# Nicolo2277/Vivim

Measured on AMD Instinct MI355X. Metric: frames/sec fwd+bwd, 256x256 clip=5 3-class, higher is better.
Workload: dtype bf16

## Files before the change

__graft_entry__.py:

```python
import os
import subprocess
import sys

ROOT = os.path.dirname(os.path.abspath(__file__))
if ROOT not in sys.path:
    sys.path.insert(0, ROOT)


def build() -> None:
    from vivim_amd import _lib
    _lib.build()
    subprocess.check_call(["make", "-C", os.path.join(ROOT, "oracle"), "-s"])
    L = _lib.lib()
    import re
    header = open(os.path.join(ROOT, "include", "vivim_hip.h")).read()
    assert L.vivim_abi_version() == int(re.search(r"#define VIVIM_ABI_VERSION (\d+)", header).group(1))
    import causal_conv1d
    import mamba_ssm
    import modeling.vivim


def smoke() -> None:
    import torch
    from mamba_ssm.ops.selective_scan_interface import mamba_inner_fn_no_out_proj
    from oracle import ref_torch
    assert torch.cuda.is_available(), "smoke() needs a GPU"
    dev = torch.device("cuda:0")
    g = torch.Generator().manual_seed(0)
    b, d_inner, n, r, L = 2, 128, 16, 4, 3 * 16 * 16
    p = dict(conv_w=torch.randn(d_inner, 1, 4, generator=g) * 0.3, conv_b=torch.randn(d_inner, generator=g) * 0.1,
             x_proj=torch.randn(r + 2 * n, d_inner, generator=g) * d_inner ** -0.5,
             dt_proj=(torch.rand(d_inner, r, generator=g) * 2 - 1) * r ** -0.5,
             A=-torch.arange(1, n + 1, dtype=torch.float32).repeat(d_inner, 1), D=torch.ones(d_inner),
             dt_bias=torch.full((d_inner,), -4.0))
    xz = torch.randn(b, 2 * d_inner, L, generator=g)
    dout = torch.randn(b, d_inner, L, generator=g)

    def run(device, fn):
        q = {k: v.to(device).requires_grad_(True) for k, v in p.items()}
        x = xz.to(device).requires_grad_(True)
        if fn is mamba_inner_fn_no_out_proj:
            y = fn(x, q["conv_w"], q["conv_b"], q["x_proj"], q["dt_proj"], q["A"], None, None, q["D"],
                   delta_bias=q["dt_bias"], delta_softplus=True)
        else:
            y = fn(x, q["conv_w"], q["conv_b"], q["x_proj"], q["dt_proj"], q["A"], q["D"], q["dt_bias"], True)
        y.backward(dout.to(device))
        return [y.detach().cpu(), x.grad.cpu()] + [q[k].grad.cpu() for k in sorted(q)]

    got = run(dev, mamba_inner_fn_no_out_proj)
    want = run("cpu", ref_torch.mamba_inner_no_out_proj_ref)
    for i, (a, w) in enumerate(zip(got, want)):
        err = float((a.double() - w.double()).norm() / w.double().norm())
        assert err < 1e-3, f"smoke: tensor {i} rel err {err:.3e}"
    torch.cuda.synchronize()
    print("smoke OK: fused inner op fwd+bwd matches the oracle (max rel err < 1e-3)")


if __name__ == "__main__":
    build()
    if len(sys.argv) > 1 and sys.argv[1] == "smoke":
        smoke()
```

vivim_amd/_lib.py:

```python
import collections
import ctypes
import os
import re
import subprocess

import torch

_HERE = os.path.dirname(os.path.abspath(__file__))
CSRC = os.path.join(_HERE, "csrc")
SO_PATH = os.environ.get("VIVIM_LIB") or os.path.join(CSRC, "libvivim_hip.so")
HEADER = os.path.join(os.path.dirname(_HERE), "include", "vivim_hip.h")
EXT_HEADER = os.path.join(os.path.dirname(_HERE), "include", "vivim_hip_ext.h")

i32, i64, vp = ctypes.c_int32, ctypes.c_int64, ctypes.c_void_p

STRUCT_NAMES = {
    "vivim_ssm_fwd_params": "SsmFwdParams", "vivim_ssm_bwd_params": "SsmBwdParams",
    "vivim_conv_fwd_params": "ConvFwdParams", "vivim_conv_bwd_params": "ConvBwdParams",
    "vivim_dwconv_params": "DwConvParams", "vivim_dwconv_wgrad_params": "DwConvWgradParams",
    "vivim_dir_params": "DirParams", "vivim_conv_update_params": "ConvUpdateParams",
    "vivim_state_update_params": "StateUpdateParams", "vivim_layernorm_params": "LayerNormParams",
    "vivim_wgrad_nt_params": "WgradNtParams", "vivim_add_layernorm_params": "AddLayerNormParams",
    "vivim_seg_loss_params": "SegLossParams", "vivim_seg_metrics_params": "SegMetricsParams",
    "vivim_upsample_params": "UpsampleParams",
    "vivim_decode_head_params": "DecodeHeadParams", "vivim_token_layernorm_params": "TokenLayerNormParams",
    "vivim_token_add_norm_params": "TokenAddNormParams", "vivim_opt_step_params": "OptStepParams",
    "vivim_opt_mw_params": "OptMwParams",
}
EXT_STRUCT_NAMES = {"vivim_structure_loss_params": "StructureLossParams"}
EXTENSIONS = {
    "vivim_hip_ext.h": (EXT_STRUCT_NAMES, {}),
    "vivim_hip_ext_head.h": ({"vivim_head_concat_params": "HeadConcatParams"}, {}),
}

Entry = collections.namedtuple("Entry", "struct extra stream restype")

_FIELD_TYPES = {"int32_t": i32, "int64_t": i64, "float": ctypes.c_float, "double": ctypes.c_double,
                "void *": vp, "const void *": vp, "const void *const *": ctypes.POINTER(vp),
                "const int64_t *": ctypes.POINTER(i64)}
_ARG_TYPES = {"void *": vp, "size_t": ctypes.c_size_t, "int": ctypes.c_int}
_RESTYPES = {"int": ctypes.c_int, "size_t": ctypes.c_size_t, "const char *": ctypes.c_char_p}
_DIRECTIVES = r"\s*#\s*(include|define|ifndef\s+VIVIM_HIP(_[A-Z0-9]+)*_H|endif)\b"


def _refuse(what, text):
    raise ValueError(f"vivim_hip.h: {what}: {' '.join(text.split())!r}")


def _ctype(text):
    return re.sub(r"\s*\*\s*", " *", " ".join(text.split()))


def _declarator(text, table, context):
    m = re.fullmatch(r"([\w\s*]*?)(\w+)\s*(?:\[\s*(\d+)\s*\])?", text.strip())
    if not m:
        _refuse("cannot parse the declarator", context)
    if _ctype(m[1]) not in table:
        _refuse(f"unknown type {_ctype(m[1])!r}", context)
    ctype = table[_ctype(m[1])]
    return m[2], (ctype * int(m[3]) if m[3] else ctype)


def _has_sizeof_row(cls):
    return cls._fields_[0][0] != "struct_bytes"


def parse_header(text, names=STRUCT_NAMES):
    text = re.sub(r"/\*.*?\*/", " ", text, flags=re.S)
    consts = {k: int(v) for k, v in re.findall(r"^[ \t]*#[ \t]*define[ \t]+(VIVIM_\w+)[ \t]+(-?\d+)[ \t]*$", text, flags=re.M)}
    by_c_name = {}

    def struct(m):
        body, c_name = m[1], m[2]
        if "{" in body or "#" in body:
            _refuse("nested braces or a preprocessor line in a struct", m[0])
        if c_name not in names:
            _refuse("a struct without a Python name in STRUCT_NAMES", c_name)
        types = {**_FIELD_TYPES, **by_c_name}
        fields = []
        for stmt in filter(None, (s.strip() for s in body.split(";"))):
            base = re.match(r"(?:const\s+)?\w+", stmt) or _refuse("cannot parse the field", stmt)
            first, *more = stmt.split(",")
            for decl in [first] + [f"{base[0]} {d}" for d in more]:
                fields.append(_declarator(decl, types, stmt))
        by_c_name[c_name] = type(names[c_name], (ctypes.Structure,), {"_fields_": fields, "__module__": __name__})
        return " "

    def enum(m):
        for item in filter(None, (s.strip() for s in m[1].split(","))):
            kv = re.fullmatch(r"(\w+)\s*=\s*(-?\d+)", item) or _refuse("cannot parse the enumerator", item)
            consts[kv[1]] = int(kv[2])
        return " "

    text = re.sub(r"typedef\s+struct\s*\{(.*?)\}\s*(\w+)\s*;", struct, text, flags=re.S)
    text = re.sub(r"(?:typedef\s+)?enum\s*\{([^{}]*)\}\s*\w*\s*;", enum, text)
    missing = [c for c in names if c not in by_c_name]
    if missing:
        _refuse("STRUCT_NAMES names structs the header does not have", ", ".join(missing))
    text = re.sub(r"^[ \t]*#[ \t]*ifdef[ \t]+__cplusplus\b.*?^[ \t]*#[ \t]*endif\b", " ", text, flags=re.S | re.M)
    for line in re.findall(r"^[ \t]*#.*$", text, flags=re.M):
        if not re.match(_DIRECTIVES, line):
            _refuse("a preprocessor line it does not know", line)
    text = re.sub(r"^[ \t]*#.*$", " ", text, flags=re.M)

    entries = {}
    for decl in filter(None, (s.strip() for s in text.split(";"))):
        m = re.fullmatch(r"([\w\s*]+?)(\w+)\s*\(([\w\s*,]*)\)", decl) or _refuse("cannot parse the declaration", decl)
        if _ctype(m[1]) not in _RESTYPES:
            _refuse(f"unknown return type {_ctype(m[1])!r}", decl)
        args = [] if m[3].strip() == "void" else [a.strip() for a in m[3].split(",")]
        stream = bool(args) and re.fullmatch(r"void\s*\*\s*stream", args[-1]) is not None
        args = args[:-1] if stream else args
        params, extra = None, []
        for k, arg in enumerate(args):
            p = re.fullmatch(r"const\s+(vivim_\w+)\s*\*\s*\w+", arg) if k == 0 else None
            if not p:
                extra.append(_declarator(arg, _ARG_TYPES, decl)[1])
            elif p[1] not in by_c_name:
                _refuse(f"unknown struct {p[1]}", decl)
            elif _has_sizeof_row(by_c_name[p[1]]):
                params = by_c_name[p[1]]
            else:
                extra.append(ctypes.POINTER(by_c_name[p[1]]))
        entries[m[2]] = Entry(params, tuple(extra), stream, _RESTYPES[_ctype(m[1])])
    return consts, {names[c]: by_c_name[c] for c in names}, entries


def _read_header(path=None):
    path = path or HEADER
    try:
        with open(path) as f:
            return f.read()
    except OSError as e:
        raise ImportError(f"{path} cannot be read ({e}): the binding is derived from it") from e


_consts, _classes, ENTRY_POINTS = parse_header(_read_header())
globals().update(_classes)
STRUCTS = tuple(c for c in _classes.values() if _has_sizeof_row(c))
EXPORTS = tuple(ENTRY_POINTS)
ABI_VERSION = _consts["VIVIM_ABI_VERSION"]
F32, F16, BF16 = _consts["VIVIM_F32"], _consts["VIVIM_F16"], _consts["VIVIM_BF16"]
OPT_CHUNK, OPT_MAX_TENSORS, OPT_STATE_WORDS = (_consts["VIVIM_OPT_" + n] for n in ("CHUNK", "MAX_TENSORS", "STATE_WORDS"))
ALL_ENTRY_POINTS = dict(ENTRY_POINTS)
for _file, (_names, _entries) in EXTENSIONS.items():
    _path = os.path.join(os.path.dirname(HEADER), _file)
    _, _ext_classes, _parsed = parse_header(_read_header(_path), _names)
    if any(_has_sizeof_row(c) for c in _ext_classes.values()) or set(_parsed) & set(ALL_ENTRY_POINTS) \
            or set(_ext_classes) & set(globals()):
        raise ImportError(f"{_path}: a struct that does not open with struct_bytes, or a name another header already declares")
    _entries.update(_parsed)
    ALL_ENTRY_POINTS.update(_parsed)
    globals().update(_ext_classes)
EXT_ENTRY_POINTS = EXTENSIONS[os.path.basename(EXT_HEADER)][1]

_lib = None


def build(force=False):
    if force:
        subprocess.check_call(["make", "-C", CSRC, "clean"])
    subprocess.check_call(["make", "-C", CSRC, "-j4"])
    return SO_PATH


def lib():
    global _lib
    if _lib is None:
        if not os.path.exists(SO_PATH):
            raise ImportError(
                f"{SO_PATH} is missing: run `python -c 'import __graft_entry__ as g; g.build()'` "
                "(or `make -C vivim_amd/csrc`). vivim_amd has no fallback path.")
        L = ctypes.CDLL(SO_PATH)
        for name, e in ALL_ENTRY_POINTS.items():
            fn = getattr(L, name)
            fn.argtypes = ([ctypes.POINTER(e.struct)] if e.struct else []) + list(e.extra) + ([vp] if e.stream else [])
            fn.restype = e.restype
        if L.vivim_abi_version() != ABI_VERSION:
            raise ImportError("libvivim_hip.so ABI version mismatch")
        for which, st in enumerate(STRUCTS):
            if L.vivim_sizeof(which) != ctypes.sizeof(st):
                raise ImportError(f"struct layout mismatch for {st.__name__}: "
                                  f"C {L.vivim_sizeof(which)} vs ctypes {ctypes.sizeof(st)}")
        _lib = L
    return _lib


_ISIZE = {F32: 4, F16: 2, BF16: 2}


def algorithmic_bytes(name, P):
    name = name.removesuffix("_det")
    f = P.f if isinstance(P, (SsmBwdParams, ConvBwdParams)) else P
    if name.startswith("vivim_opt"):
        if name.endswith("finalise"):
            return 8 * P.total_blocks + 4 * OPT_STATE_WORDS
        n = sum(P.numel[i] for i in range(P.count) if P.grads[i])
        if name.endswith("_mw"):
            return 2 * n + 8 * P.n_blocks if name.endswith("stats_mw") else 28 * n
        return 4 * n + 8 * P.n_blocks if name.endswith("stats") else 28 * n
    if name.startswith("vivim_add_layernorm"):
        n = P.batch * P.seqlen * P.channels
        if not P.weight:
            return n * ((2 if name.endswith("fwd") else 1) * _ISIZE[P.itype] + _ISIZE[P.btype])
        if name.endswith("fwd"):
            return n * (2 * _ISIZE[P.itype] + _ISIZE[P.btype] + _ISIZE[P.otype]) + 8 * P.batch * P.seqlen + 8 * P.channels
        res = (_ISIZE[P.itype] if P.dres else 0) + (_ISIZE[P.otype] if P.dy else 0) + (_ISIZE[P.btype] if P.dbranch else 0)
        return n * (2 * _ISIZE[P.itype] + res) + 8 * P.batch * P.seqlen + 12 * P.channels
    if name.startswith("vivim_token_add_norm"):
        n, b, r = P.rows * P.channels, _ISIZE[P.btype], _ISIZE[P.rtype]
        stats = 8 * P.rows if P.mean and P.weight else 0
        small = (4 * (P.rows // P.rows_per_sample) if P.scale else 0) + (4 * P.channels if P.weight else 0)
        if name.endswith("fwd"):
            small += 4 * P.channels if P.weight and P.bias else 0
            return n * (b + (r if P.res else 0) + (r if P.res_out else 0) + (b if P.weight else 0)) + stats + small
        norm = bool(P.weight and P.dy)
        small += (4 * P.channels if norm and P.dweight else 0) + (4 * P.channels if norm and P.dbias else 0)
        return (n * ((r + b if norm else 0) + (r if P.dres else 0) + (r if P.dres_in else 0) + (b if P.dbranch else 0))
                + (stats if norm else 0) + small)
    if name.startswith("vivim_token_layernorm"):
        n = P.rows * P.channels
        stats = 8 * P.rows if P.mean else 0
        if name.endswith("fwd"):
            return n * (_ISIZE[P.itype] + _ISIZE[P.otype]) + stats
        return n * (2 * _ISIZE[P.itype] + _ISIZE[P.otype]) + stats + 12 * P.channels
    if name.startswith("vivim_decode_head"):
        px = sum(P.map_h[s] * P.map_w[s] for s in range(P.n_maps))
        return (P.batch * (px * P.hidden + P.classes * P.out_h * P.out_w) * _ISIZE[P.itype]
                + 4 * (P.hidden + P.classes * P.hidden + P.classes))
    if name.startswith("vivim_head_concat"):
        px = P.out_h * P.out_w
        maps = sum(P.map_c[s] * (P.map_h[s] * P.map_w[s] + px) for s in range(P.n_maps)) * _ISIZE[P.itype]
        return P.batch * (maps + sum(P.map_c[s] * px for s in range(P.n_maps) if P.keep[s]))
    if name.startswith("vivim_upsample"):
        return P.batch * P.channels * (P.in_h * P.in_w + P.out_h * P.out_w) * _ISIZE[P.itype]
    if name.startswith("vivim_seg_metrics"):
        n = P.batch * P.pixels
        return n * (P.classes * _ISIZE[P.itype] + (8 if P.ttype == 0 else 1) + (1 if P.pred else 0)) + 12 * P.batch * P.classes
    if name.startswith("vivim_structure_loss"):
        n = P.batch * P.height * P.width
        return (n * ((2 if name.endswith("bwd") else 1) * P.classes * _ISIZE[P.itype] + (8 if P.ttype == 0 else 1))
                + 12 * P.batch * P.classes)
    if name.startswith("vivim_seg_loss"):
        n = P.batch * P.pixels
        return (n * ((2 if name.endswith("bwd") else 1) * P.classes * _ISIZE[P.itype] + (8 if P.ttype == 0 else 1))
                + 8 * P.batch * P.classes)
    if name.startswith("vivim_binary_metrics"):
        n = P.batch * P.height * P.width
        return (3 * n * (_ISIZE[P.ptype] + _ISIZE.get(P.gtype, 1)) + P.batch * (72 + (4096 if P.hist else 0))
                + (160 if P.state else 0))
    if name.startswith("vivim_selective_scan"):
        s = _ISIZE[f.itype]
        act = f.batch * f.dim * f.seqlen * s
        bc = (f.batch * f.n_groups * f.dstate * f.seqlen) if f.is_variable_B else f.dim * f.dstate
        has_z = bool(f.z)
        if name.endswith("fwd_lean"):
            return (4 if has_z else 3) * act + 2 * bc * (s if f.is_variable_B else 4) + 4 * (f.dim * f.dstate + 2 * f.dim)
        if name.endswith("fwd"):
            n_act = 3 + (2 if has_z else 0)
            return n_act * act + 2 * bc * (s if f.is_variable_B else 4) + 4 * (f.dim * f.dstate + 2 * f.dim)
        n_act = 5 + (3 if has_z else 0) + (1 if (has_z and f.out_z) else 0)
        return (n_act * act + 2 * bc * (s if f.is_variable_B else 4) + 2 * bc * 4
                + 4 * (2 * f.dim * f.dstate + 4 * f.dim))
    if name.endswith("_update"):
        return 0
    if name.startswith("vivim_dir"):
        return 4 * P.batch * P.channels * P.seqlen * _ISIZE[P.itype]
    if name.startswith("vivim_dwconv"):
        act = P.batch * P.depth * P.height * P.width * P.channels * _ISIZE[P.itype]
        return 2 * act + 4 * P.channels * (P.kd * 9 + 1)
    if name.startswith("vivim_layernorm"):
        n = P.batch * P.seqlen * P.channels
        if name.endswith("fwd"):
            return n * (_ISIZE[P.itype] + _ISIZE[P.otype]) + 8 * P.batch * P.seqlen + 8 * P.channels
        return n * (2 * _ISIZE[P.itype] + _ISIZE[P.otype]) + 8 * P.batch * P.seqlen + 12 * P.channels
    if name.startswith("vivim_wgrad"):
        return P.groups * ((P.m + P.n) * P.k * _ISIZE[P.itype] + 4 * P.m * P.n)
    s = _ISIZE[f.itype]
    act = f.batch * f.dim * f.seqlen * s
    if name.endswith("fwd"):
        return 2 * act + 4 * f.dim * (f.width + 1)
    return 3 * act + 8 * f.dim * (f.width + 1)


_profile = None
_event_pool = []
_PROFILED = ("vivim_selective_scan_fwd", "vivim_selective_scan_bwd", "vivim_causal_conv1d_fwd",
             "vivim_causal_conv1d_bwd")


def profile_begin(all_kernels=False):
    global _profile
    _profile = ([], bool(all_kernels))


def profile_end():
    global _profile
    rec = _profile[0] if _profile else []
    _profile = None
    out = []
    for name, nbytes, e0, e1 in rec:
        e1.synchronize()
        out.append((name, nbytes, e0.elapsed_time(e1) * 1e-3))
        _event_pool.extend((e0, e1))
    return out


def _event():
    if _event_pool:
        return _event_pool.pop()
    return torch.cuda.Event(enable_timing=True)


GUARD = os.environ.get("VIVIM_GUARD", "0") not in ("0", "")
_GUARD_BYTES = 1 << 16
_guards = []


def _guarded_storage(nbytes, device):
    buf = torch.full((nbytes + 2 * _GUARD_BYTES,), 0xA5, dtype=torch.uint8, device=device)
    _guards.append(buf)
    return buf[_GUARD_BYTES:_GUARD_BYTES + nbytes]


def empty(shape, dtype, device):
    if not GUARD:
        return torch.empty(shape, dtype=dtype, device=device)
    n = 1
    for d in shape:
        n *= d
    return _guarded_storage(n * torch.empty((), dtype=dtype).element_size(), device).view(dtype).view(shape)


def zeros(n, device):
    if not GUARD:
        return torch.zeros(n, dtype=torch.float32, device=device)
    return _guarded_storage(4 * n, device).view(torch.float32).zero_()


def empty_like(t):
    if not GUARD:
        return torch.empty_like(t)
    ref = torch.empty_like(t)
    flat = _guarded_storage(t.numel() * t.element_size(), t.device).view(t.dtype)
    return flat.as_strided(ref.shape, ref.stride())


def check_guards(what):
    torch.cuda.synchronize()
    for buf in _guards:
        lo, hi = buf[:_GUARD_BYTES], buf[-_GUARD_BYTES:]
        if not (bool((lo == 0xA5).all()) and bool((hi == 0xA5).all())):
            nlo, nhi = int((lo != 0xA5).sum()), int((hi != 0xA5).sum())
            _guards.clear()
            raise RuntimeError(f"VIVIM_GUARD: {what} wrote outside a {buf.numel() - 2 * _GUARD_BYTES}-byte buffer "
                               f"({nlo} bytes below, {nhi} bytes above)")
    _guards.clear()


def deterministic():
    return torch.are_deterministic_algorithms_enabled()


def call(name, params, stream, *extra):
    L = lib()
    fn = getattr(L, name)
    if _profile is not None and (_profile[1] or name in _PROFILED):
        e0, e1 = _event(), _event()
        e0.record()
        rc = fn(ctypes.byref(params), *extra, stream)
        e1.record()
        _profile[0].append((name, algorithmic_bytes(name, params), e0, e1))
    else:
        rc = fn(ctypes.byref(params), *extra, stream)
    if rc != 0:
        raise RuntimeError(L.vivim_last_error().decode())
    if GUARD:
        check_guards(name)


def launch(name, params, device, *extra):
    if device.index == torch.cuda.current_device():
        call(name, params, torch.cuda.current_stream().cuda_stream, *extra)
    else:
        with torch.cuda.device(device):
            call(name, params, torch.cuda.current_stream().cuda_stream, *extra)


ITYPE = {torch.float32: F32, torch.float16: F16, torch.bfloat16: BF16}


def ptr(t):
    return None if t is None else t.data_ptr()


def check(cond, msg):
    if not cond:
        raise RuntimeError(msg)


def workspace(query, params, device):
    n = getattr(lib(), query)(params)
    return n, (empty((n,), torch.uint8, device) if n else None)
```

vivim_amd/csrc/capi.hip:

```cpp
#include <hip/hip_runtime.h>
#include <float.h>
#include <stdarg.h>
#include <stddef.h>
#include <stdio.h>
#include <string.h>
#include <type_traits>
#include "ops.cuh"

using vivim::Launch;
using vivim::conv_channel_last;
using vivim::elem_bytes;
using vivim::vec_elems;

static thread_local char g_err[512] = "";

static int fail(int code, const char* fmt, ...) {
    va_list ap;
    va_start(ap, fmt);
    vsnprintf(g_err, sizeof(g_err), fmt, ap);
    va_end(ap);
    return code;
}

#define VCHECK(cond)                                                                   \
    do {                                                                               \
        if (!(cond)) return fail(VIVIM_ERR_INVALID, "%s: check failed: %s", __func__, #cond); \
    } while (0)

static int after_launch(const char* what) {
    const hipError_t e = hipGetLastError();
    if (e != hipSuccess) return fail(VIVIM_ERR_LAUNCH, "%s: launch failed: %s", what, hipGetErrorString(e));
    return VIVIM_OK;
}

static bool dtype_ok(int t) { return t == VIVIM_F32 || t == VIVIM_F16 || t == VIVIM_BF16; }
static bool aligned(const void* q, uintptr_t bytes) { return reinterpret_cast<uintptr_t>(q) % bytes == 0; }
static bool aligned16(const void* q) { return aligned(q, 16); }
static hipStream_t as_stream(void* stream) { return static_cast<hipStream_t>(stream); }

static int bad_workspace(const char* fn, const char* query, long long bytes, const void* at, int align, size_t need) {
    return fail(VIVIM_ERR_INVALID, "%s: workspace of %lld bytes at %p: need a %d-byte aligned one of %s() = %zu", fn, bytes, at, align,
                query, need);
}
static int check_workspace(const char* fn, const char* query, const void* ws, int64_t bytes, int align, size_t need) {
    if (ws == nullptr || !aligned(ws, align) || bytes < 0 || (size_t)bytes < need) return bad_workspace(fn, query, bytes, ws, align, need);
    return VIVIM_OK;
}
static int check_struct_bytes(const char* fn, const char* name, int32_t struct_bytes, size_t size) {
    if (struct_bytes != (int32_t)size)
        return fail(VIVIM_ERR_INVALID, "%s: struct_bytes = %d, this library's %s has %zu", fn, struct_bytes, name, size);
    return VIVIM_OK;
}

enum SsmCheck { kSsmFwd, kSsmBwd, kSsmFwdLean };
static int check_ssm_fwd(const vivim_ssm_fwd_params* p, SsmCheck mode) {
    const bool is_bwd = mode == kSsmBwd;
    VCHECK(p != nullptr);
    VCHECK(dtype_ok(p->itype));
    VCHECK(p->batch > 0 && p->dim > 0 && p->seqlen > 0 && p->dstate > 0 && p->n_groups > 0);
    VCHECK(p->dstate <= 256);
    VCHECK(p->dim % p->n_groups == 0);
    VCHECK(p->u && p->delta && p->A && p->B && p->C);
    if (mode == kSsmFwdLean) {
        if (p->x != nullptr)
            return fail(VIVIM_ERR_INVALID, "selective_scan_fwd_lean: x must be NULL (this entry point writes no checkpoints; "
                        "vivim_selective_scan_fwd is the call that fills x)");
        if (p->z) {
            VCHECK(p->out_z != nullptr);
            if (p->out != nullptr)
                return fail(VIVIM_ERR_INVALID, "selective_scan_fwd_lean: with z only out_z is written, out must be NULL");
        } else {
            VCHECK(p->out != nullptr);
        }
    } else {
        VCHECK(p->x != nullptr || (is_bwd && p->seqlen <= vivim::scan_ckpt_len(*p)));
        if (!is_bwd) VCHECK(p->out != nullptr);
        if (p->z) {
            if (!is_bwd) VCHECK(p->out_z != nullptr);
            else VCHECK(p->out != nullptr);
        }
    }
    if (p->is_variable_B != p->is_variable_C)
        return fail(VIVIM_ERR_UNSUPPORTED,
                    "selective_scan: mixed constant/variable B and C is not built (Vivim uses variable B and C)");
    if (!p->is_variable_B) VCHECK(p->n_groups == 1);
    return VIVIM_OK;
}

template <class P> static int check_seg_inputs(const P* p, const char* name) {
    VCHECK(p != nullptr);
    VCHECK(dtype_ok(p->itype) && (p->ttype == 0 || p->ttype == 1));
    VCHECK(p->batch > 0 && p->pixels > 0);
    if (p->classes < 2 || p->classes > 8)
        return fail(VIVIM_ERR_UNSUPPORTED, "%s: %d classes: the kernels are built for 2 to 8 classes", name, p->classes);
    if constexpr (std::is_same<P, vivim_seg_loss_params>::value)
        if (p->gamma != 2.0f)
            return fail(VIVIM_ERR_UNSUPPORTED, "seg_loss: gamma = %g: the kernels are built for gamma = 2 only", (double)p->gamma);
    VCHECK((int64_t)p->batch * 64 <= INT32_MAX);
    VCHECK(p->logits && aligned(p->logits, p->itype == VIVIM_F32 ? 4 : 2));
    VCHECK(p->target && aligned(p->target, p->ttype == 0 ? 8 : 1));
    return VIVIM_OK;
}

namespace vivim {
static int g_tune[2] = {-1, -1};
static int tuning_get(int which, const char* env) {
    int v = __atomic_load_n(&g_tune[which], __ATOMIC_RELAXED);
    if (v < 0) {
        const char* e = getenv(env);
        v = e ? atoi(e) : 0;
        if (v < 0) v = 0;
        __atomic_store_n(&g_tune[which], v, __ATOMIC_RELAXED);
    }
    return v;
}
int tuning_fwd_variant() { return tuning_get(0, "VIVIM_FWD_VARIANT"); }
int tuning_bwd_variant() { return tuning_get(1, "VIVIM_BWD_VARIANT"); }
}

extern "C" {

int vivim_set_tuning(int which, int value) {
    if (which < 0 || which > 1 || value < 0) return -1;
    const int prev = which == 0 ? vivim::tuning_fwd_variant() : vivim::tuning_bwd_variant();
    __atomic_store_n(&vivim::g_tune[which], value, __ATOMIC_RELAXED);
    return prev;
}
int vivim_abi_version(void) { return VIVIM_ABI_VERSION; }
const char* vivim_last_error(void) { return g_err; }
int vivim_scan_chunk_len(int itype) { return vivim::scan_chunk_len(itype); }
int vivim_scan_ckpt_len(const vivim_ssm_fwd_params* f) { return f ? vivim::scan_ckpt_len(*f) : 0; }
size_t vivim_scan_bwd_workspace_bytes(const vivim_ssm_fwd_params* f) {
    return f ? vivim::scan_bwd_workspace_bytes(*f) : 0;
}
size_t vivim_scan_fwd_workspace_bytes(const vivim_ssm_fwd_params* f) {
    return f ? vivim::scan_fwd_workspace_bytes(*f) : 0;
}
size_t vivim_sizeof(int which) {
    static const size_t sizes[] = {
        sizeof(vivim_ssm_fwd_params), sizeof(vivim_ssm_bwd_params), sizeof(vivim_conv_fwd_params), sizeof(vivim_conv_bwd_params),
        sizeof(vivim_dwconv_params), sizeof(vivim_dwconv_wgrad_params), sizeof(vivim_dir_params), sizeof(vivim_conv_update_params),
        sizeof(vivim_state_update_params), sizeof(vivim_layernorm_params), sizeof(vivim_wgrad_nt_params),
        sizeof(vivim_add_layernorm_params), sizeof(vivim_seg_loss_params), sizeof(vivim_seg_metrics_params),
        sizeof(vivim_upsample_params)};
    return which >= 0 && which < (int)(sizeof(sizes) / sizeof(sizes[0])) ? sizes[which] : 0;
}

int vivim_selective_scan_fwd(const vivim_ssm_fwd_params* p, void* stream) {
    if (int rc = check_ssm_fwd(p, kSsmFwd)) return rc;
    if (!vivim::ssm_fwd_dispatch(*p, as_stream(stream)))
        return fail(VIVIM_ERR_UNSUPPORTED, "selective_scan_fwd not implemented for input type %d", p->itype);
    return after_launch("selective_scan_fwd");
}

int vivim_selective_scan_fwd_lean(const vivim_ssm_fwd_params* p, void* last_state, void* stream) {
    if (int rc = check_ssm_fwd(p, kSsmFwdLean)) return rc;
    if (!vivim::ssm_fwd_lean_dispatch(*p, last_state, as_stream(stream)))
        return fail(VIVIM_ERR_UNSUPPORTED, "selective_scan_fwd_lean not implemented for input type %d", p->itype);
    return after_launch("selective_scan_fwd_lean");
}

static int check_ssm_bwd(const vivim_ssm_bwd_params* p) {
    VCHECK(p != nullptr);
    if (int rc = check_ssm_fwd(&p->f, kSsmBwd)) return rc;
    VCHECK(p->dout && p->du && p->ddelta && p->dA && p->dB && p->dC);
    VCHECK((p->f.D == nullptr) == (p->dD == nullptr));
    VCHECK((p->f.delta_bias == nullptr) == (p->ddelta_bias == nullptr));
    VCHECK((p->f.z == nullptr) == (p->dz == nullptr));
    return VIVIM_OK;
}

int vivim_selective_scan_bwd(const vivim_ssm_bwd_params* p, void* stream) {
    if (int rc = check_ssm_bwd(p)) return rc;
    if (!vivim::ssm_bwd_dispatch(*p, as_stream(stream)))
        return fail(VIVIM_ERR_UNSUPPORTED, "selective_scan_bwd not implemented for input type %d", p->f.itype);
    return after_launch("selective_scan_bwd");
}

size_t vivim_scan_bwd_det_workspace_bytes(const vivim_ssm_fwd_params* f) {
    return f && f->batch > 0 && f->dim > 0 && f->seqlen > 0 && f->dstate > 0 && f->n_groups > 0
               ? vivim::scan_bwd_det_workspace_bytes(*f) : 0;
}

size_t vivim_scan_bwd_det_call_workspace_bytes(const vivim_ssm_bwd_params* p) {
    return check_ssm_bwd(p) == VIVIM_OK ? vivim::scan_bwd_det_call_workspace_bytes(*p) : 0;
}

int vivim_selective_scan_bwd_det(const vivim_ssm_bwd_params* p, void* det_ws, size_t det_ws_bytes, void* stream) {
    if (int rc = check_ssm_bwd(p)) return rc;
    switch (vivim::ssm_bwd_det_dispatch(*p, det_ws, det_ws_bytes, as_stream(stream))) {
        case Launch::ok: break;
        case Launch::bad_workspace:
            return bad_workspace("selective_scan_bwd_det", "vivim_scan_bwd_det_call_workspace_bytes", det_ws_bytes, det_ws, 16,
                                 vivim::scan_bwd_det_call_workspace_bytes(*p));
        case Launch::unsupported: return fail(VIVIM_ERR_UNSUPPORTED, "selective_scan_bwd_det not implemented for input type %d", p->f.itype);
    }
    return after_launch("selective_scan_bwd_det");
}

static int check_conv(const vivim_conv_fwd_params* p) {
    VCHECK(p != nullptr);
    VCHECK(dtype_ok(p->itype) && dtype_ok(p->wtype));
    VCHECK(p->batch > 0 && p->dim > 0 && p->seqlen > 0);
    VCHECK(p->batch <= 65535 && p->dim <= 65535);
    if (!(p->width >= 2 && p->width <= 4))
        return fail(VIVIM_ERR_INVALID, "causal_conv1d only supports width between 2 and 4");
    VCHECK(p->x && p->weight);
    if (p->x_l_stride != 1 && p->x_c_stride != 1)
        return fail(VIVIM_ERR_INVALID, "causal_conv1d: x must have unit stride along seqlen or along channels");
    return VIVIM_OK;
}

int vivim_causal_conv1d_fwd(const vivim_conv_fwd_params* p, void* stream) {
    if (int rc = check_conv(p)) return rc;
    VCHECK(p->out != nullptr);
    const bool cl = conv_channel_last(*p);
    if (cl) { VCHECK(p->out_c_stride == 1); } else { VCHECK(p->out_l_stride == 1); }
    if (!vivim::conv_fwd_dispatch(*p, as_stream(stream)))
        return fail(VIVIM_ERR_UNSUPPORTED, "causal_conv1d_fwd not implemented for input type %d / weight type %d",
                    p->itype, p->wtype);
    return after_launch("causal_conv1d_fwd");
}

static int check_conv_bwd(const vivim_conv_bwd_params* p) {
    VCHECK(p != nullptr);
    if (int rc = check_conv(&p->f)) return rc;
    VCHECK(p->dout && p->dx && p->dweight);
    const bool cl = conv_channel_last(p->f);
    if (cl) { VCHECK(p->dout_c_stride == 1 && p->dx_c_stride == 1); }
    else    { VCHECK(p->dout_l_stride == 1 && p->dx_l_stride == 1); }
    VCHECK((p->f.bias == nullptr) == (p->dbias == nullptr));
    return VIVIM_OK;
}

size_t vivim_causal_conv1d_bwd_det_workspace_bytes(const vivim_conv_fwd_params* f) {
    return check_conv(f) == VIVIM_OK ? vivim::conv_bwd_det_workspace_bytes(*f) : 0;
}

int vivim_causal_conv1d_bwd_det(const vivim_conv_bwd_params* p, void* det_ws, size_t det_ws_bytes, void* stream) {
    if (int rc = check_conv_bwd(p)) return rc;
    switch (vivim::conv_bwd_det_dispatch(*p, det_ws, det_ws_bytes, as_stream(stream))) {
        case Launch::ok: break;
        case Launch::bad_workspace:
            return bad_workspace("causal_conv1d_bwd_det", "vivim_causal_conv1d_bwd_det_workspace_bytes", det_ws_bytes, det_ws, 16,
                                 vivim::conv_bwd_det_workspace_bytes(p->f));
        case Launch::unsupported:
            return fail(VIVIM_ERR_UNSUPPORTED, "causal_conv1d_bwd_det not implemented for input type %d / weight type %d",
                        p->f.itype, p->f.wtype);
    }
    return after_launch("causal_conv1d_bwd_det");
}

int vivim_causal_conv1d_bwd(const vivim_conv_bwd_params* p, void* stream) {
    if (int rc = check_conv_bwd(p)) return rc;
    if (!vivim::conv_bwd_dispatch(*p, as_stream(stream)))
        return fail(VIVIM_ERR_UNSUPPORTED, "causal_conv1d_bwd not implemented for input type %d / weight type %d",
                    p->f.itype, p->f.wtype);
    return after_launch("causal_conv1d_bwd");
}

static int check_dw_dims(int batch, int depth, int height, int width, int channels, int kd, int itype) {
    VCHECK(dtype_ok(itype));
    VCHECK(batch > 0 && depth > 0 && height > 0 && width > 0 && channels > 0);
    VCHECK(kd == 1 || kd == 3);
    VCHECK(batch <= 65535);
    return VIVIM_OK;
}

int vivim_dwconv_fwd(const vivim_dwconv_params* p, void* stream) {
    VCHECK(p != nullptr);
    if (int rc = check_dw_dims(p->batch, p->depth, p->height, p->width, p->channels, p->kd, p->itype)) return rc;
    VCHECK(p->x && p->wt && p->y);
    const int64_t cv = vec_elems(p->itype);
    VCHECK(p->channels % cv == 0 && p->x_token_stride % cv == 0 && p->x_batch_stride % cv == 0 &&
           p->y_token_stride % cv == 0 && p->y_batch_stride % cv == 0);
    VCHECK(aligned16(p->x) && aligned16(p->y));
    VCHECK(p->act >= 0 && p->act <= 2 && (p->act == 0 || p->flip == 0));
    if (p->act == 2)
        VCHECK(p->aux && aligned16(p->aux) && p->aux_token_stride % cv == 0 &&
               p->aux_batch_stride % cv == 0);
    if (!vivim::dwconv_fwd_dispatch(*p, as_stream(stream)))
        return fail(VIVIM_ERR_UNSUPPORTED, "dwconv_fwd not implemented for input type %d", p->itype);
    return after_launch("dwconv_fwd");
}

static int check_dw_wgrad(const vivim_dwconv_wgrad_params* p) {
    VCHECK(p != nullptr);
    if (int rc = check_dw_dims(p->batch, p->depth, p->height, p->width, p->channels, p->kd, p->itype)) return rc;
    VCHECK(p->x && p->dy && p->dwt);
    VCHECK(p->channels % 2 == 0 && p->x_token_stride % 2 == 0 && p->x_batch_stride % 2 == 0 &&
           p->dy_token_stride % 2 == 0 && p->dy_batch_stride % 2 == 0);
    VCHECK(aligned(p->x, 8) && aligned(p->dy, 8));
    return VIVIM_OK;
}

size_t vivim_dwconv_wgrad_det_workspace_bytes(const vivim_dwconv_wgrad_params* p) {
    if (!p || p->batch <= 0 || p->depth <= 0 || p->height <= 0 || p->width <= 0 || p->channels <= 0 || (p->kd != 1 && p->kd != 3))
        return 0;
    return vivim::dwconv_wgrad_det_workspace_bytes(*p);
}

int vivim_dwconv_wgrad_det(const vivim_dwconv_wgrad_params* p, void* det_ws, size_t det_ws_bytes, void* stream) {
    if (int rc = check_dw_wgrad(p)) return rc;
    switch (vivim::dwconv_wgrad_det_dispatch(*p, det_ws, det_ws_bytes, as_stream(stream))) {
        case Launch::ok: break;
        case Launch::bad_workspace:
            return bad_workspace("dwconv_wgrad_det", "vivim_dwconv_wgrad_det_workspace_bytes", det_ws_bytes, det_ws, 16,
                                 vivim::dwconv_wgrad_det_workspace_bytes(*p));
        case Launch::unsupported: return fail(VIVIM_ERR_UNSUPPORTED, "dwconv_wgrad_det not implemented for input type %d", p->itype);
    }
    return after_launch("dwconv_wgrad_det");
}

int vivim_dwconv_wgrad(const vivim_dwconv_wgrad_params* p, void* stream) {
    if (int rc = check_dw_wgrad(p)) return rc;
    if (!vivim::dwconv_wgrad_dispatch(*p, as_stream(stream)))
        return fail(VIVIM_ERR_UNSUPPORTED, "dwconv_wgrad not implemented for input type %d", p->itype);
    return after_launch("dwconv_wgrad");
}

static int check_dir(const vivim_dir_params* p) {
    VCHECK(p != nullptr);
    VCHECK(p->itype == VIVIM_F32 || p->itype == VIVIM_F16 || p->itype == VIVIM_BF16);
    VCHECK(p->batch > 0 && p->channels > 0 && p->seqlen > 0 && p->nframes > 0 && p->csplit > 0);
    VCHECK(p->batch <= 65535 && p->channels <= 65535);
    VCHECK(p->seqlen % p->nframes == 0 && p->channels % p->csplit == 0);
    VCHECK(p->src && p->dst);
    const int64_t e = vec_elems(p->itype);
    VCHECK(p->seqlen % e == 0);
    VCHECK(aligned16(p->src) && aligned16(p->dst));
    VCHECK(p->flat_batch_stride % e == 0 && p->flat_c_stride % e == 0 && p->stk_batch_stride % e == 0 &&
           p->stk_half_stride % e == 0 && p->stk_dir_stride % e == 0 && p->stk_c_stride % e == 0);
    return VIVIM_OK;
}

int vivim_dir_scatter(const vivim_dir_params* p, void* stream) {
    if (int rc = check_dir(p)) return rc;
    if (!vivim::dir_dispatch<false>(*p, as_stream(stream))) return fail(VIVIM_ERR_UNSUPPORTED, "dir_scatter: bad itype");
    return after_launch("dir_scatter");
}

int vivim_dir_gather(const vivim_dir_params* p, void* stream) {
    if (int rc = check_dir(p)) return rc;
    if (!vivim::dir_dispatch<true>(*p, as_stream(stream))) return fail(VIVIM_ERR_UNSUPPORTED, "dir_gather: bad itype");
    return after_launch("dir_gather");
}

int vivim_causal_conv1d_update(const vivim_conv_update_params* p, void* stream) {
    VCHECK(p != nullptr);
    VCHECK(dtype_ok(p->itype) && dtype_ok(p->wtype));
    VCHECK(p->batch > 0 && p->dim > 0 && p->batch <= 65535);
    if (p->width < 2 || p->width > 4)
        return fail(VIVIM_ERR_UNSUPPORTED, "causal_conv1d only supports width between 2 and 4");
    VCHECK(p->x && p->conv_state && p->weight && p->out);
    vivim::conv_update_launch(*p, as_stream(stream));
    return after_launch("causal_conv1d_update");
}

int vivim_selective_state_update(const vivim_state_update_params* p, void* stream) {
    VCHECK(p != nullptr);
    VCHECK(dtype_ok(p->itype) && (p->stype == VIVIM_F32 || p->stype == p->itype));
    VCHECK(p->batch > 0 && p->dim > 0 && p->dstate > 0 && p->batch <= 65535);
    VCHECK(p->state && p->x && p->dt && p->A && p->B && p->C && p->out);
    vivim::state_update_launch(*p, as_stream(stream));
    return after_launch("selective_state_update");
}

static int check_layernorm(const vivim_layernorm_params* p) {
    VCHECK(p != nullptr);
    VCHECK(dtype_ok(p->itype) && (p->otype == VIVIM_F32 || p->otype == p->itype));
    VCHECK(p->batch > 0 && p->seqlen > 0 && p->channels > 0 && p->batch <= 65535);
    if (p->channels > 512)
        return fail(VIVIM_ERR_UNSUPPORTED, "layernorm_cm: more than 512 channels do not fit the backward's two LDS tiles");
    const int64_t e = vec_elems(p->itype);
    VCHECK(p->seqlen % e == 0 && p->x_batch_stride % e == 0 && p->x_c_stride % e == 0);
    VCHECK(p->x && aligned16(p->x) && p->mean && p->rstd);
    return VIVIM_OK;
}

int vivim_layernorm_cm_fwd(const vivim_layernorm_params* p, void* stream) {
    if (int rc = check_layernorm(p)) return rc;
    VCHECK(p->y != nullptr);
    if (!vivim::layernorm_dispatch(*p, false, as_stream(stream)))
        return fail(VIVIM_ERR_UNSUPPORTED, "layernorm_cm_fwd not implemented for input type %d / output type %d", p->itype, p->otype);
    return after_launch("layernorm_cm_fwd");
}

size_t vivim_layernorm_bwd_workspace_bytes(const vivim_layernorm_params* p) {
    return p && p->batch > 0 && p->seqlen > 0 && p->channels > 0 ? vivim::layernorm_bwd_workspace_bytes(*p) : 0;
}

int vivim_layernorm_cm_bwd(const vivim_layernorm_params* p, void* stream) {
    if (int rc = check_layernorm(p)) return rc;
    VCHECK(p->dy && p->dx && aligned16(p->dx));
    const int64_t e = vec_elems(p->itype);
    VCHECK(p->dx_batch_stride % e == 0 && p->dx_c_stride % e == 0);
    if ((p->dweight || p->dbias) && !p->workspace)
        return fail(VIVIM_ERR_INVALID, "layernorm_cm_bwd: dweight / dbias need the workspace (vivim_layernorm_bwd_workspace_bytes)");
    if (!vivim::layernorm_dispatch(*p, true, as_stream(stream)))
        return fail(VIVIM_ERR_UNSUPPORTED, "layernorm_cm_bwd not implemented for input type %d / output type %d", p->itype, p->otype);
    return after_launch("layernorm_cm_bwd");
}

int vivim_wgrad_nt(const vivim_wgrad_nt_params* p, void* stream) {
    VCHECK(p != nullptr);
    VCHECK(p->groups > 0 && p->groups <= 65535 && p->m > 0 && p->n > 0 && p->k > 0);
    VCHECK(p->a && p->b && p->out);
    if (p->itype != VIVIM_F16 && p->itype != VIVIM_BF16)
        return fail(VIVIM_ERR_UNSUPPORTED, "wgrad_nt takes f16 or bf16 operands (type %d given): f32 products stay on the library GEMM", p->itype);
    VCHECK(p->k % 8 == 0 && p->a_row_stride % 8 == 0 && p->b_row_stride % 8 == 0 && p->a_group_stride % 8 == 0 &&
           p->b_group_stride % 8 == 0);
    VCHECK(aligned16(p->a) && aligned16(p->b));
    VCHECK((int64_t)((p->m + 63) / 64) * ((p->n + 15) / 16) <= 65535);
    if (!vivim::wgrad_nt_dispatch(*p, as_stream(stream)))
        return fail(VIVIM_ERR_UNSUPPORTED, "wgrad_nt not implemented for type %d", p->itype);
    return after_launch("wgrad_nt");
}

static int check_add_layernorm(const vivim_add_layernorm_params* p, int64_t* e) {
    VCHECK(p != nullptr);
    VCHECK(dtype_ok(p->itype) && dtype_ok(p->btype) && (p->weight == nullptr || dtype_ok(p->otype)));
    VCHECK(p->batch > 0 && p->seqlen > 0 && p->channels > 0 && p->batch <= 65535);
    if (p->channels > 512)
        return fail(VIVIM_ERR_UNSUPPORTED, "add_layernorm_cm: more than 512 channels do not fit the backward's two LDS tiles");
    if (p->btype != p->itype && p->itype != VIVIM_F32)
        return fail(VIVIM_ERR_UNSUPPORTED, "add_layernorm_cm: branch type %d with x type %d is not built (the branch has x's type, or x is f32)",
                    p->btype, p->itype);
    if (p->weight && p->otype != VIVIM_F32 && p->otype != p->itype)
        return fail(VIVIM_ERR_UNSUPPORTED, "add_layernorm_cm: output type %d with x type %d is not built (f32 or x's type)", p->otype, p->itype);
    *e = vec_elems(p->itype);
    VCHECK(p->seqlen % *e == 0);
    return VIVIM_OK;
}

int vivim_add_layernorm_cm_fwd(const vivim_add_layernorm_params* p, void* stream) {
    int64_t e = 0;
    if (int rc = check_add_layernorm(p, &e)) return rc;
    VCHECK(p->x && p->branch && p->x_new && aligned16(p->x) && aligned16(p->x_new));
    VCHECK(p->x_batch_stride % e == 0 && p->x_c_stride % e == 0 && p->x_new_batch_stride % e == 0 && p->x_new_c_stride % e == 0);
    if (p->weight) VCHECK(p->y && p->mean && p->rstd);
    if (!vivim::add_layernorm_dispatch(*p, false, as_stream(stream)))
        return fail(VIVIM_ERR_UNSUPPORTED, "add_layernorm_cm_fwd not implemented for x type %d / branch type %d / output type %d", p->itype,
                    p->btype, p->otype);
    return after_launch("add_layernorm_cm_fwd");
}

size_t vivim_add_layernorm_bwd_workspace_bytes(const vivim_add_layernorm_params* p) {
    return p && p->batch > 0 && p->seqlen > 0 && p->channels > 0 ? vivim::add_layernorm_bwd_workspace_bytes(*p) : 0;
}

int vivim_add_layernorm_cm_bwd(const vivim_add_layernorm_params* p, void* stream) {
    int64_t e = 0;
    if (int rc = check_add_layernorm(p, &e)) return rc;
    if (p->dres) VCHECK(aligned16(p->dres) && p->dres_batch_stride % e == 0 && p->dres_c_stride % e == 0);
    if (p->weight) {
        VCHECK(p->x_new && aligned16(p->x_new) && p->mean && p->rstd && (p->dy || p->dres));
        VCHECK(p->x_new_batch_stride % e == 0 && p->x_new_c_stride % e == 0);
        VCHECK(p->dx && aligned16(p->dx) && p->dx_batch_stride % e == 0 && p->dx_c_stride % e == 0);
        if ((p->dweight || p->dbias) && !p->workspace)
            return fail(VIVIM_ERR_INVALID,
                        "add_layernorm_cm_bwd: dweight / dbias need the workspace (vivim_add_layernorm_bwd_workspace_bytes)");
    } else {
        VCHECK(p->dres && p->dbranch);
    }
    if (!vivim::add_layernorm_dispatch(*p, true, as_stream(stream)))
        return fail(VIVIM_ERR_UNSUPPORTED, "add_layernorm_cm_bwd not implemented for x type %d / branch type %d / output type %d", p->itype,
                    p->btype, p->otype);
    return after_launch("add_layernorm_cm_bwd");
}

static int check_seg_loss(const vivim_seg_loss_params* p) {
    if (int rc = check_seg_inputs(p, "seg_loss")) return rc;
    VCHECK(p->alpha && aligned(p->alpha, 4));
    return VIVIM_OK;
}

size_t vivim_seg_loss_workspace_bytes(const vivim_seg_loss_params* p) {
    return p && p->batch > 0 && p->pixels > 0 && p->classes > 0 && dtype_ok(p->itype) ? vivim::seg_loss_workspace_bytes(*p) : 0;
}

int vivim_seg_loss_fwd(const vivim_seg_loss_params* p, void* stream) {
    if (int rc = check_seg_loss(p)) return rc;
    VCHECK(p->loss && aligned(p->loss, 4));
    VCHECK(aligned(p->coef, 4));
    const size_t need = vivim::seg_loss_workspace_bytes(*p);
    if (int rc = check_workspace("seg_loss_fwd", "vivim_seg_loss_workspace_bytes", p->workspace, p->workspace_bytes, 4, need)) return rc;
    if (!vivim::seg_loss_dispatch(*p, false, as_stream(stream)))
        return fail(VIVIM_ERR_UNSUPPORTED, "seg_loss_fwd not implemented for input type %d / %d classes", p->itype, p->classes);
    return after_launch("seg_loss_fwd");
}

int vivim_seg_loss_bwd(const vivim_seg_loss_params* p, void* stream) {
    if (int rc = check_seg_loss(p)) return rc;
    const uintptr_t ib = elem_bytes(p->itype);
    VCHECK(p->coef && aligned(p->coef, 4));
    VCHECK(p->grad_out && aligned(p->grad_out, 4));
    VCHECK(p->dlogits && aligned(p->dlogits, ib));
    if (!vivim::seg_loss_dispatch(*p, true, as_stream(stream)))
        return fail(VIVIM_ERR_UNSUPPORTED, "seg_loss_bwd not implemented for input type %d / %d classes", p->itype, p->classes);
    return after_launch("seg_loss_bwd");
}

size_t vivim_seg_metrics_workspace_bytes(const vivim_seg_metrics_params* p) {
    return p && p->batch > 0 && p->pixels > 0 && p->classes > 0 && dtype_ok(p->itype) ? vivim::seg_metrics_workspace_bytes(*p) : 0;
}

int vivim_seg_metrics(const vivim_seg_metrics_params* p, void* stream) {
    if (int rc = check_seg_inputs(p, "seg_metrics")) return rc;
    VCHECK(p->counts && aligned(p->counts, 4));
    VCHECK(aligned(p->state, 8));
    const size_t need = vivim::seg_metrics_workspace_bytes(*p);
    if (int rc = check_workspace("seg_metrics", "vivim_seg_metrics_workspace_bytes", p->workspace, p->workspace_bytes, 4, need)) return rc;
    if (!vivim::seg_metrics_dispatch(*p, as_stream(stream)))
        return fail(VIVIM_ERR_UNSUPPORTED, "seg_metrics not implemented for input type %d / %d classes", p->itype, p->classes);
    return after_launch("seg_metrics");
}

static int check_upsample(const vivim_upsample_params* p, bool bwd) {
    VCHECK(p != nullptr);
    VCHECK(dtype_ok(p->itype) && (p->layout == 0 || p->layout == 1));
    VCHECK(p->batch > 0 && p->channels > 0 && p->in_h > 0 && p->in_w > 0 && p->out_h > 0 && p->out_w > 0);
    if (p->out_h < p->in_h || p->out_w < p->in_w)
        return fail(VIVIM_ERR_UNSUPPORTED, "upsample_bilinear2d: (%d, %d) -> (%d, %d): upsampling only", p->in_h, p->in_w, p->out_h,
                    p->out_w);
    const uintptr_t ib = elem_bytes(p->itype);
    const void* src = bwd ? p->dy : p->x;
    const void* dst = bwd ? p->dx : p->y;
    VCHECK(src != nullptr && aligned(src, ib));
    VCHECK(dst != nullptr && aligned(dst, ib));
    VCHECK((int64_t)p->channels * p->in_h * p->in_w <= INT32_MAX && (int64_t)p->channels * p->out_h * p->out_w <= INT32_MAX);
    VCHECK((2 * (int64_t)p->in_h + 3) * p->out_h <= INT32_MAX && (2 * (int64_t)p->in_w + 3) * p->out_w <= INT32_MAX);
    VCHECK((int64_t)p->batch * p->channels <= INT32_MAX && (int64_t)p->batch * p->out_h <= INT32_MAX);
    VCHECK(vivim::upsample_blocks(*p, bwd) <= INT32_MAX);
    return VIVIM_OK;
}

int vivim_upsample_bilinear2d_fwd(const vivim_upsample_params* p, void* stream) {
    if (int rc = check_upsample(p, false)) return rc;
    if (!vivim::upsample_dispatch(*p, false, as_stream(stream)))
        return fail(VIVIM_ERR_UNSUPPORTED, "upsample_bilinear2d_fwd not implemented for type %d", p->itype);
    return after_launch("upsample_bilinear2d_fwd");
}

int vivim_upsample_bilinear2d_bwd(const vivim_upsample_params* p, void* stream) {
    if (int rc = check_upsample(p, true)) return rc;
    if (!vivim::upsample_dispatch(*p, true, as_stream(stream)))
        return fail(VIVIM_ERR_UNSUPPORTED, "upsample_bilinear2d_bwd not implemented for type %d", p->itype);
    return after_launch("upsample_bilinear2d_bwd");
}

static int check_decode_head(const vivim_decode_head_params* p) {
    VCHECK(p != nullptr);
    if (int rc = check_struct_bytes("decode_head_fwd", "vivim_decode_head_params", p->struct_bytes, sizeof(*p))) return rc;
    VCHECK(dtype_ok(p->itype));
    VCHECK(p->batch > 0 && p->hidden > 0 && p->classes > 0 && p->out_h > 0 && p->out_w > 0);
    VCHECK(p->n_maps >= 1 && p->n_maps <= 4);
    VCHECK(p->classes <= 8);
    if (p->hidden > vivim::decode_head_max_hidden())
        return fail(VIVIM_ERR_INVALID, "decode_head_fwd: hidden = %d: bias and w_out are kept in LDS, which holds up to %d channels",
                    p->hidden, vivim::decode_head_max_hidden());
    const uintptr_t ib = elem_bytes(p->itype);
    VCHECK((int64_t)p->classes * p->out_h * p->out_w <= INT32_MAX);
    for (int s = 0; s < p->n_maps; ++s) {
        VCHECK(p->map_h[s] > 0 && p->map_w[s] > 0);
        if (p->map_h[s] > p->out_h || p->map_w[s] > p->out_w)
            return fail(VIVIM_ERR_UNSUPPORTED, "decode_head_fwd: map %d is (%d, %d), the output (%d, %d): upsampling only", s, p->map_h[s],
                        p->map_w[s], p->out_h, p->out_w);
        VCHECK((int64_t)p->hidden * p->map_h[s] * p->map_w[s] <= INT32_MAX);
    }
    for (int s = 0; s < p->n_maps; ++s) VCHECK(p->maps[s] != nullptr && aligned(p->maps[s], ib));
    VCHECK(p->bias != nullptr && aligned(p->bias, 4));
    VCHECK(p->w_out != nullptr && aligned(p->w_out, 4));
    VCHECK(aligned(p->b_out, 4));
    VCHECK(p->logits != nullptr && aligned(p->logits, ib));
    for (int s = 0; s < p->n_maps; ++s) VCHECK(p->map_batch_stride[s] >= (int64_t)p->hidden * p->map_h[s] * p->map_w[s]);
    VCHECK(p->logits_batch_stride >= (int64_t)p->classes * p->out_h * p->out_w);
    VCHECK(vivim::decode_head_blocks(*p) <= INT32_MAX);
    return VIVIM_OK;
}

int vivim_decode_head_fwd(const vivim_decode_head_params* p, void* stream) {
    if (int rc = check_decode_head(p)) return rc;
    if (!vivim::decode_head_dispatch(*p, as_stream(stream)))
        return fail(VIVIM_ERR_UNSUPPORTED, "decode_head_fwd not implemented for type %d", p->itype);
    return after_launch("decode_head_fwd");
}

static int check_token_layernorm(const vivim_token_layernorm_params* p, const char* fn) {
    VCHECK(p != nullptr);
    if (int rc = check_struct_bytes(fn, "vivim_token_layernorm_params", p->struct_bytes, sizeof(*p))) return rc;
    VCHECK(dtype_ok(p->itype) && dtype_ok(p->otype));
    VCHECK(p->rows > 0);
    if (p->channels < 1)
        return fail(VIVIM_ERR_INVALID, "%s: channels = %d: a row has at least one channel", fn, p->channels);
    if (p->channels > 1024)
        return fail(VIVIM_ERR_UNSUPPORTED, "%s: channels = %d: a row of more than 1024 channels does not fit the lanes' registers", fn,
                    p->channels);
    if (!vivim::token_layernorm_pair_ok(p->itype, p->otype))
        return fail(VIVIM_ERR_UNSUPPORTED, "%s: input type %d with output type %d is not built (the same type, an f32 output, or an f32 input)",
                    fn, p->itype, p->otype);
    VCHECK(p->x != nullptr && aligned(p->x, p->itype == VIVIM_F32 ? 4 : 2));
    VCHECK(p->weight != nullptr && aligned(p->weight, 4));
    if (p->x_row_stride < p->channels)
        return fail(VIVIM_ERR_INVALID, "%s: x_row_stride = %lld is less than the %d channels of a row", fn, (long long)p->x_row_stride,
                    p->channels);
    return VIVIM_OK;
}

int vivim_token_layernorm_fwd(const vivim_token_layernorm_params* p, void* stream) {
    if (int rc = check_token_layernorm(p, "token_layernorm_fwd")) return rc;
    VCHECK(p->y != nullptr && aligned(p->y, p->otype == VIVIM_F32 ? 4 : 2));
    VCHECK(aligned(p->bias, 4));
    VCHECK((p->mean == nullptr) == (p->rstd == nullptr) && aligned(p->mean, 4) && aligned(p->rstd, 4));
    if (p->y_row_stride < p->channels)
        return fail(VIVIM_ERR_INVALID, "token_layernorm_fwd: y_row_stride = %lld is less than the %d channels of a row",
                    (long long)p->y_row_stride, p->channels);
    if (!vivim::token_layernorm_dispatch(*p, false, as_stream(stream)))
        return fail(VIVIM_ERR_UNSUPPORTED, "token_layernorm_fwd not implemented for input type %d / output type %d", p->itype, p->otype);
    return after_launch("token_layernorm_fwd");
}

size_t vivim_token_layernorm_bwd_workspace_bytes(const vivim_token_layernorm_params* p) {
    return p && p->rows > 0 && p->channels > 0 && p->channels <= 1024 ? vivim::token_layernorm_bwd_workspace_bytes(*p) : 0;
}

int vivim_token_layernorm_bwd(const vivim_token_layernorm_params* p, void* stream) {
    if (int rc = check_token_layernorm(p, "token_layernorm_bwd")) return rc;
    VCHECK(p->dy != nullptr && aligned(p->dy, p->otype == VIVIM_F32 ? 4 : 2));
    VCHECK(p->dx != nullptr && aligned(p->dx, p->itype == VIVIM_F32 ? 4 : 2));
    VCHECK(p->mean != nullptr && p->rstd != nullptr && aligned(p->mean, 4) && aligned(p->rstd, 4));
    VCHECK(aligned(p->dweight, 4) && aligned(p->dbias, 4) && aligned(p->workspace, 4));
    if (p->dy_row_stride < p->channels || p->dx_row_stride < p->channels)
        return fail(VIVIM_ERR_INVALID, "token_layernorm_bwd: dy_row_stride = %lld / dx_row_stride = %lld is less than the %d channels of a row",
                    (long long)p->dy_row_stride, (long long)p->dx_row_stride, p->channels);
    if ((p->dweight || p->dbias) && !p->workspace)
        return fail(VIVIM_ERR_INVALID, "token_layernorm_bwd: dweight / dbias need the workspace (vivim_token_layernorm_bwd_workspace_bytes)");
    if (!vivim::token_layernorm_dispatch(*p, true, as_stream(stream)))
        return fail(VIVIM_ERR_UNSUPPORTED, "token_layernorm_bwd not implemented for input type %d / output type %d", p->itype, p->otype);
    return after_launch("token_layernorm_bwd");
}

static int check_token_add_norm(const vivim_token_add_norm_params* p, const char* fn) {
    VCHECK(p != nullptr);
    if (int rc = check_struct_bytes(fn, "vivim_token_add_norm_params", p->struct_bytes, sizeof(*p))) return rc;
    if (!dtype_ok(p->btype) || !dtype_ok(p->rtype) || !dtype_ok(p->otype))
        return fail(VIVIM_ERR_INVALID, "%s: btype = %d, rtype = %d, otype = %d: a type tag is 0 (f32), 1 (f16) or 2 (bf16)", fn, p->btype,
                    p->rtype, p->otype);
    if (p->rows <= 0) return fail(VIVIM_ERR_INVALID, "%s: rows = %d: at least one row", fn, p->rows);
    if (p->channels < 1)
        return fail(VIVIM_ERR_INVALID, "%s: channels = %d: a row has at least one channel", fn, p->channels);
    if (p->channels > 1024)
        return fail(VIVIM_ERR_UNSUPPORTED, "%s: channels = %d: a row of more than 1024 channels does not fit the lanes' registers", fn,
                    p->channels);
    if (!vivim::token_add_norm_pair_ok(p->btype, p->rtype) || p->otype != p->btype)
        return fail(VIVIM_ERR_UNSUPPORTED, "%s: branch type %d with residual type %d and output type %d is not built (one type, or an "
                    "f16 / bf16 branch and output on an f32 residual)", fn, p->btype, p->rtype, p->otype);
    if (p->rms != 0 && p->rms != 1) return fail(VIVIM_ERR_INVALID, "%s: rms = %d: 0 (LayerNorm) or 1 (RMSNorm)", fn, p->rms);
    if (p->scale != nullptr && (p->rows_per_sample <= 0 || p->rows % p->rows_per_sample != 0))
        return fail(VIVIM_ERR_INVALID, "%s: rows_per_sample = %d with scale: it must be positive and divide rows = %d", fn,
                    p->rows_per_sample, p->rows);
    return VIVIM_OK;
}

static int check_tan_tensor(const char* fn, const char* name, const void* q, bool required, int type, int64_t stride, int channels) {
    if (q == nullptr)
        return required ? fail(VIVIM_ERR_INVALID, "%s: %s is NULL", fn, name) : VIVIM_OK;
    if (!aligned(q, elem_bytes(type)))
        return fail(VIVIM_ERR_INVALID, "%s: %s = %p is not aligned to its element type", fn, name, q);
    if (stride < channels)
        return fail(VIVIM_ERR_INVALID, "%s: %s_row_stride = %lld is less than the %d channels of a row", fn, name, (long long)stride, channels);
    return VIVIM_OK;
}
static int check_tan_f32(const char* fn, const char* name, const void* q, bool required) {
    if (q == nullptr)
        return required ? fail(VIVIM_ERR_INVALID, "%s: %s is NULL", fn, name) : VIVIM_OK;
    return aligned(q, 4) ? VIVIM_OK : fail(VIVIM_ERR_INVALID, "%s: %s = %p is not aligned to its element type", fn, name, q);
}

int vivim_token_add_norm_fwd(const vivim_token_add_norm_params* p, void* stream) {
    const char* fn = "token_add_norm_fwd";
    if (int rc = check_token_add_norm(p, fn)) return rc;
    const bool norm = p->weight != nullptr;
    const int C = p->channels;
    if (int rc = check_tan_tensor(fn, "branch", p->branch, true, p->btype, p->branch_row_stride, C)) return rc;
    if (int rc = check_tan_tensor(fn, "res", p->res, false, p->rtype, p->res_row_stride, C)) return rc;
    if (int rc = check_tan_tensor(fn, "res_out", p->res_out, !norm || p->res != nullptr, p->rtype, p->res_out_row_stride, C)) return rc;
    if (int rc = check_tan_f32(fn, "scale", p->scale, false)) return rc;
    if (norm) {
        if (int rc = check_tan_tensor(fn, "y", p->y, true, p->otype, p->y_row_stride, C)) return rc;
        if (int rc = check_tan_f32(fn, "weight", p->weight, true)) return rc;
        if (int rc = check_tan_f32(fn, "bias", p->bias, false)) return rc;
        if ((p->mean == nullptr) != (p->rstd == nullptr))
            return fail(VIVIM_ERR_INVALID, "%s: mean = %p with rstd = %p: both or neither", fn, p->mean, p->rstd);
        if (int rc = check_tan_f32(fn, "mean", p->mean, false)) return rc;
        if (int rc = check_tan_f32(fn, "rstd", p->rstd, false)) return rc;
    }
    if (!vivim::token_add_norm_dispatch(*p, false, as_stream(stream)))
        return fail(VIVIM_ERR_UNSUPPORTED, "%s not implemented for branch type %d / residual type %d", fn, p->btype, p->rtype);
    return after_launch(fn);
}

size_t vivim_token_add_norm_bwd_workspace_bytes(const vivim_token_add_norm_params* p) {
    return p && p->rows > 0 && p->channels > 0 && p->channels <= 1024 ? vivim::token_add_norm_bwd_workspace_bytes(*p) : 0;
}

int vivim_token_add_norm_bwd(const vivim_token_add_norm_params* p, void* stream) {
    const char* fn = "token_add_norm_bwd";
    if (int rc = check_token_add_norm(p, fn)) return rc;
    const bool norm = p->weight != nullptr;
    const int C = p->channels;
    if (p->dy == nullptr && p->dres == nullptr) return fail(VIVIM_ERR_INVALID, "%s: dy and dres are both NULL: nothing to propagate", fn);
    if (!norm && p->dy != nullptr) return fail(VIVIM_ERR_INVALID, "%s: dy = %p without weight: the add alone has no y", fn, p->dy);
    if (norm) {
        if (int rc = check_tan_tensor(fn, "res_out", p->res_out, true, p->rtype, p->res_out_row_stride, C)) return rc;
        if (int rc = check_tan_f32(fn, "mean", p->mean, true)) return rc;
        if (int rc = check_tan_f32(fn, "rstd", p->rstd, true)) return rc;
        if (int rc = check_tan_f32(fn, "weight", p->weight, true)) return rc;
        if (int rc = check_tan_tensor(fn, "dy", p->dy, false, p->otype, p->dy_row_stride, C)) return rc;
        if (int rc = check_tan_f32(fn, "dweight", p->dweight, false)) return rc;
        if (int rc = check_tan_f32(fn, "dbias", p->dbias, false)) return rc;
        if (int rc = check_tan_f32(fn, "workspace", p->workspace, false)) return rc;
        if ((p->dweight || p->dbias) && !p->workspace)
            return fail(VIVIM_ERR_INVALID, "%s: dweight / dbias need the workspace (vivim_token_add_norm_bwd_workspace_bytes)", fn);
    }
    if (int rc = check_tan_tensor(fn, "dres", p->dres, false, p->rtype, p->dres_row_stride, C)) return rc;
    if (int rc = check_tan_tensor(fn, "dres_in", p->dres_in, false, p->rtype, p->dres_in_row_stride, C)) return rc;
    if (int rc = check_tan_tensor(fn, "dbranch", p->dbranch, false, p->btype, p->dbranch_row_stride, C)) return rc;
    if (int rc = check_tan_f32(fn, "scale", p->scale, false)) return rc;
    if (!vivim::token_add_norm_dispatch(*p, true, as_stream(stream)))
        return fail(VIVIM_ERR_UNSUPPORTED, "%s not implemented for branch type %d / residual type %d", fn, p->btype, p->rtype);
    return after_launch(fn);
}

static int check_opt_common(const vivim_opt_step_params* p, const char* fn) {
    VCHECK(p != nullptr);
    if (int rc = check_struct_bytes(fn, "vivim_opt_step_params", p->struct_bytes, sizeof(*p))) return rc;
    VCHECK(p->state != nullptr && aligned(p->state, 4));
    if (p->total_blocks < 0) return fail(VIVIM_ERR_INVALID, "%s: total_blocks = %d", fn, p->total_blocks);
    return VIVIM_OK;
}

static int check_opt_tensors(const vivim_opt_step_params* p, const char* fn, size_t grad_align = 4) {
    if (p->count <= 0 || p->count > VIVIM_OPT_MAX_TENSORS)
        return fail(VIVIM_ERR_INVALID, "%s: count = %d, a call takes 1 to %d tensors", fn, p->count, VIVIM_OPT_MAX_TENSORS);
    VCHECK(p->grads != nullptr && p->numel != nullptr && p->block_map != nullptr);
    VCHECK(aligned(p->block_map, 4) && p->first_tensor >= 0);
    for (int i = 0; i < p->count; ++i) {
        if (p->numel[i] <= 0) return fail(VIVIM_ERR_INVALID, "%s: numel[%d] = %lld", fn, i, (long long)p->numel[i]);
        VCHECK(aligned(p->grads[i], grad_align));
    }
    if (p->first_block < 0 || p->n_blocks <= 0 || (int64_t)p->first_block + p->n_blocks > p->total_blocks)
        return fail(VIVIM_ERR_INVALID, "%s: map rows %d .. %d + %d of %d", fn, p->first_block, p->first_block, p->n_blocks, p->total_blocks);
    return VIVIM_OK;
}

static int check_opt_workspace(const vivim_opt_step_params* p, const char* fn) {
    const size_t need = 8 * (size_t)p->total_blocks;
    if (need && (p->workspace == nullptr || !aligned(p->workspace, 8) || p->workspace_bytes < (int64_t)need))
        return bad_workspace(fn, "vivim_opt_step_workspace_bytes", (long long)p->workspace_bytes, p->workspace, 8, need);
    return VIVIM_OK;
}

static int check_opt_hyper(const vivim_opt_step_params* p, const char* fn, bool update) {
    if (!(p->beta1 >= 0.0 && p->beta1 < 1.0 && p->beta2 >= 0.0 && p->beta2 < 1.0))
        return fail(VIVIM_ERR_INVALID, "%s: betas = (%g, %g), each must be in [0, 1)", fn, p->beta1, p->beta2);
    if (update && !(p->lr >= 0.0 && p->eps >= 0.0 && p->weight_decay >= 0.0))
        return fail(VIVIM_ERR_INVALID, "%s: lr = %g, eps = %g, weight_decay = %g: none may be negative", fn, p->lr, p->eps, p->weight_decay);
    return VIVIM_OK;
}

size_t vivim_opt_step_workspace_bytes(const vivim_opt_step_params* p) {
    return p && p->struct_bytes == (int32_t)sizeof(vivim_opt_step_params) && p->total_blocks > 0 ? 8 * (size_t)p->total_blocks : 0;
}

int vivim_opt_grad_stats(const vivim_opt_step_params* p, void* stream) {
    const char* fn = "opt_grad_stats";
    if (int rc = check_opt_common(p, fn)) return rc;
    if (int rc = check_opt_tensors(p, fn)) return rc;
    if (int rc = check_opt_workspace(p, fn)) return rc;
    vivim::opt_grad_stats_launch(*p, as_stream(stream));
    return after_launch(fn);
}

int vivim_opt_finalise(const vivim_opt_step_params* p, void* stream) {
    const char* fn = "opt_finalise";
    if (int rc = check_opt_common(p, fn)) return rc;
    if (int rc = check_opt_hyper(p, fn, false)) return rc;
    if (p->has_max_norm && !(p->max_norm >= 0.0)) return fail(VIVIM_ERR_INVALID, "%s: max_norm = %g", fn, p->max_norm);
    if (int rc = check_opt_workspace(p, fn)) return rc;
    vivim::opt_finalise_launch(*p, as_stream(stream));
    return after_launch(fn);
}

int vivim_opt_adamw(const vivim_opt_step_params* p, void* stream) {
    const char* fn = "opt_adamw";
    if (int rc = check_opt_common(p, fn)) return rc;
    VCHECK(p->params != nullptr && p->exp_avg != nullptr && p->exp_avg_sq != nullptr);
    VCHECK(aligned(p->params, 8) && aligned(p->exp_avg, 8) && aligned(p->exp_avg_sq, 8));
    if (int rc = check_opt_tensors(p, fn)) return rc;
    if (int rc = check_opt_hyper(p, fn, true)) return rc;
    vivim::opt_adamw_launch(*p, as_stream(stream));
    return after_launch(fn);
}

static int check_opt_mw(const vivim_opt_mw_params* p, const char* fn, vivim_opt_step_params& q) {
    VCHECK(p != nullptr);
    if (int rc = check_struct_bytes(fn, "vivim_opt_mw_params", p->struct_bytes, sizeof(*p))) return rc;
    static_assert(offsetof(vivim_opt_mw_params, masters) == sizeof(vivim_opt_step_params), "the common fields come first");
    memcpy(&q, p, sizeof(q));
    q.struct_bytes = (int32_t)sizeof(q);
    if (int rc = check_opt_common(&q, fn)) return rc;
    if (p->dtype != VIVIM_F16 && p->dtype != VIVIM_BF16)
        return fail(VIVIM_ERR_INVALID, "%s: dtype = %d, master weights are for 1 (fp16) and 2 (bf16)", fn, p->dtype);
    return VIVIM_OK;
}

int vivim_opt_grad_stats_mw(const vivim_opt_mw_params* p, void* stream) {
    const char* fn = "opt_grad_stats_mw";
    vivim_opt_step_params q;
    if (int rc = check_opt_mw(p, fn, q)) return rc;
    if (int rc = check_opt_tensors(&q, fn, 2)) return rc;
    if (int rc = check_opt_workspace(&q, fn)) return rc;
    vivim::opt_grad_stats_mw_launch(q, p->dtype, as_stream(stream));
    return after_launch(fn);
}

int vivim_opt_adamw_mw(const vivim_opt_mw_params* p, void* stream) {
    const char* fn = "opt_adamw_mw";
    vivim_opt_step_params q;
    if (int rc = check_opt_mw(p, fn, q)) return rc;
    VCHECK(q.params != nullptr && q.exp_avg != nullptr && q.exp_avg_sq != nullptr && p->masters != nullptr);
    VCHECK(aligned(q.params, 8) && aligned(q.exp_avg, 8) && aligned(q.exp_avg_sq, 8) && aligned(p->masters, 8));
    if (int rc = check_opt_tensors(&q, fn, 2)) return rc;
    if (int rc = check_opt_hyper(&q, fn, true)) return rc;
    vivim::opt_adamw_mw_launch(q, p->masters, p->dtype, as_stream(stream));
    return after_launch(fn);
}


static bool structure_loss_sizes_ok(const vivim_structure_loss_params* p) {
    return p->batch > 0 && p->classes > 0 && p->height > 0 && p->width > 0;
}

static int check_structure_loss(const vivim_structure_loss_params* p, const char* fn) {
    if (p == nullptr) return fail(VIVIM_ERR_INVALID, "%s: params is NULL", fn);
    if (int rc = check_struct_bytes(fn, "vivim_structure_loss_params", p->struct_bytes, sizeof(*p))) return rc;
    if (!dtype_ok(p->itype) || (p->ttype != 0 && p->ttype != 1))
        return fail(VIVIM_ERR_INVALID, "%s: itype = %d, ttype = %d: logits are fp32 / fp16 / bf16 (0 / 1 / 2), targets int64 / uint8 (0 / 1)",
                    fn, p->itype, p->ttype);
    if (!structure_loss_sizes_ok(p))
        return fail(VIVIM_ERR_INVALID, "%s: batch = %d, classes = %d, height = %d, width = %d: every size must be positive", fn, p->batch,
                    p->classes, p->height, p->width);
    if (p->classes > 8)
        return fail(VIVIM_ERR_UNSUPPORTED, "%s: %d classes: the kernels are built for 1 to 8 classes", fn, p->classes);
    if (p->first_class < 0 || p->first_class > 255)
        return fail(VIVIM_ERR_INVALID, "%s: first_class = %d: labels are compared as values in [0, 256)", fn, p->first_class);
    if ((int64_t)p->height * p->width > INT32_MAX - 4096 || (int64_t)p->batch * vivim::structure_loss_tiles(*p) > INT32_MAX)
        return fail(VIVIM_ERR_INVALID, "%s: batch = %d, height = %d, width = %d: the index range overflows int32", fn, p->batch, p->height,
                    p->width);
    const uintptr_t ib = elem_bytes(p->itype);
    if (p->logits == nullptr || !aligned(p->logits, ib))
        return fail(VIVIM_ERR_INVALID, "%s: logits at %p: need a %d-byte aligned pointer", fn, p->logits, (int)ib);
    if (p->target == nullptr || !aligned(p->target, p->ttype == 0 ? 8 : 1))
        return fail(VIVIM_ERR_INVALID, "%s: target at %p: need a %d-byte aligned pointer", fn, p->target, p->ttype == 0 ? 8 : 1);
    return VIVIM_OK;
}

size_t vivim_structure_loss_workspace_bytes(const vivim_structure_loss_params* p) {
    if (p == nullptr || p->struct_bytes != (int32_t)sizeof(vivim_structure_loss_params) || !structure_loss_sizes_ok(p) || p->classes > 8 ||
        !dtype_ok(p->itype))
        return 0;
    return vivim::structure_loss_workspace_bytes(*p);
}

int vivim_structure_loss_fwd(const vivim_structure_loss_params* p, void* stream) {
    const char* fn = "structure_loss_fwd";
    if (int rc = check_structure_loss(p, fn)) return rc;
    if (p->loss == nullptr || !aligned(p->loss, 4)) return fail(VIVIM_ERR_INVALID, "%s: loss at %p: need a 4-byte aligned pointer", fn, p->loss);
    if (!aligned(p->coef, 4))
        return fail(VIVIM_ERR_INVALID, "%s: coef at %p: need a 4-byte aligned pointer (or NULL)", fn, p->coef);
    const size_t need = vivim::structure_loss_workspace_bytes(*p);
    if (int rc = check_workspace(fn, "vivim_structure_loss_workspace_bytes", p->workspace, p->workspace_bytes, 8, need)) return rc;
    if (!vivim::structure_loss_dispatch(*p, false, as_stream(stream)))
        return fail(VIVIM_ERR_UNSUPPORTED, "%s not implemented for input type %d", fn, p->itype);
    return after_launch(fn);
}

int vivim_structure_loss_bwd(const vivim_structure_loss_params* p, void* stream) {
    const char* fn = "structure_loss_bwd";
    if (int rc = check_structure_loss(p, fn)) return rc;
    const uintptr_t ib = elem_bytes(p->itype);
    if (p->coef == nullptr || !aligned(p->coef, 4)) return fail(VIVIM_ERR_INVALID, "%s: coef at %p: need a 4-byte aligned pointer", fn, p->coef);
    if (p->grad_out == nullptr || !aligned(p->grad_out, 4))
        return fail(VIVIM_ERR_INVALID, "%s: grad_out at %p: need a 4-byte aligned pointer", fn, p->grad_out);
    if (p->dlogits == nullptr || !aligned(p->dlogits, ib))
        return fail(VIVIM_ERR_INVALID, "%s: dlogits at %p: need a %d-byte aligned pointer", fn, p->dlogits, (int)ib);
    if (!vivim::structure_loss_dispatch(*p, true, as_stream(stream)))
        return fail(VIVIM_ERR_UNSUPPORTED, "%s not implemented for input type %d", fn, p->itype);
    return after_launch(fn);
}


static int check_head_concat(const vivim_head_concat_params* p, const char* fn, bool bwd) {
    if (p == nullptr) return fail(VIVIM_ERR_INVALID, "%s: params is NULL", fn);
    if (int rc = check_struct_bytes(fn, "vivim_head_concat_params", p->struct_bytes, sizeof(*p))) return rc;
    if (p->n_maps < 1 || p->n_maps > 4) return fail(VIVIM_ERR_INVALID, "%s: n_maps = %d: one to four maps", fn, p->n_maps);
    if (!dtype_ok(p->itype)) return fail(VIVIM_ERR_INVALID, "%s: itype = %d: the maps are fp32 / fp16 / bf16 (0 / 1 / 2)", fn, p->itype);
    if (p->batch <= 0 || p->out_h <= 0 || p->out_w <= 0)
        return fail(VIVIM_ERR_INVALID, "%s: batch = %d, out_h = %d, out_w = %d: every size must be positive", fn, p->batch, p->out_h, p->out_w);
    for (int s = 0; s < p->n_maps; ++s)
        if (p->map_c[s] <= 0 || p->map_h[s] <= 0 || p->map_w[s] <= 0)
            return fail(VIVIM_ERR_INVALID, "%s: map %d: map_c = %d, map_h = %d, map_w = %d: every size must be positive", fn, s, p->map_c[s],
                        p->map_h[s], p->map_w[s]);
    for (int s = 0; s < p->n_maps; ++s)
        if (p->map_h[s] > p->out_h || p->map_w[s] > p->out_w)
            return fail(VIVIM_ERR_UNSUPPORTED, "%s: map %d is (%d, %d), the output (%d, %d): upsampling only", fn, s, p->map_h[s], p->map_w[s],
                        p->out_h, p->out_w);
    for (int s = 0; s < p->n_maps; ++s) {
        if (p->chan_off[s] < 0 || (int64_t)p->chan_off[s] + p->map_c[s] > p->out_pixel_stride)
            return fail(VIVIM_ERR_INVALID, "%s: map %d: channels [%d, %lld) lie outside a pixel of out_pixel_stride = %lld", fn, s, p->chan_off[s],
                        (long long)p->chan_off[s] + p->map_c[s], (long long)p->out_pixel_stride);
        for (int t = 0; t < s; ++t)
            if (p->chan_off[s] < p->chan_off[t] + p->map_c[t] && p->chan_off[t] < p->chan_off[s] + p->map_c[s])
                return fail(VIVIM_ERR_INVALID, "%s: the channel blocks of maps %d and %d overlap: [%d, %d) and [%d, %d)", fn, t, s, p->chan_off[t],
                            p->chan_off[t] + p->map_c[t], p->chan_off[s], p->chan_off[s] + p->map_c[s]);
    }
    const uintptr_t ib = elem_bytes(p->itype);
    const void* big = bwd ? p->dout : p->out;
    if (big == nullptr || !aligned(big, ib))
        return fail(VIVIM_ERR_INVALID, "%s: %s at %p: need a %d-byte aligned pointer", fn, bwd ? "dout" : "out", big, (int)ib);
    for (int s = 0; s < p->n_maps; ++s) {
        const void* q = bwd ? p->dmaps[s] : p->maps[s];
        if (q == nullptr || !aligned(q, ib))
            return fail(VIVIM_ERR_INVALID, "%s: %s[%d] at %p: need a %d-byte aligned pointer", fn, bwd ? "dmaps" : "maps", s, q, (int)ib);
    }
    for (int s = 0; s < p->n_maps; ++s)
        if (!(p->scale[s] >= 1.0f) || p->scale[s] > FLT_MAX)
            return fail(VIVIM_ERR_INVALID, "%s: scale[%d] = %g: 1 / (1 - p) is finite and at least 1", fn, s, (double)p->scale[s]);
    const int64_t out_image = (int64_t)p->out_h * p->out_w * p->out_pixel_stride;
    if (p->out_batch_stride < out_image)
        return fail(VIVIM_ERR_INVALID, "%s: out_batch_stride = %lld: an image of out has %lld elements", fn, (long long)p->out_batch_stride,
                    (long long)out_image);
    for (int s = 0; s < p->n_maps; ++s) {
        const int64_t image = (int64_t)p->map_c[s] * p->map_h[s] * p->map_w[s], mask = (int64_t)p->map_c[s] * p->out_h * p->out_w;
        const int64_t have = bwd ? p->dmap_batch_stride[s] : p->map_batch_stride[s];
        if (have < image)
            return fail(VIVIM_ERR_INVALID, "%s: %s[%d] = %lld: an image of map %d has %lld elements", fn,
                        bwd ? "dmap_batch_stride" : "map_batch_stride", s, (long long)have, s, (long long)image);
        if (p->keep[s] != nullptr && p->keep_batch_stride[s] < mask)
            return fail(VIVIM_ERR_INVALID, "%s: keep_batch_stride[%d] = %lld: a mask of map %d has %lld bytes", fn, s,
                        (long long)p->keep_batch_stride[s], s, (long long)mask);
    }
    bool fits = out_image <= INT32_MAX - 256 && (int64_t)p->batch * p->out_h <= INT32_MAX;
    for (int s = 0; s < p->n_maps; ++s)
        fits = fits && (2 * (int64_t)p->map_h[s] + 3) * p->out_h <= INT32_MAX && (2 * (int64_t)p->map_w[s] + 3) * p->out_w <= INT32_MAX;
    if (!fits || vivim::head_concat_blocks(*p, bwd) > INT32_MAX)
        return fail(VIVIM_ERR_INVALID, "%s: batch = %d, out (%d, %d), out_pixel_stride = %lld: the index range overflows int32", fn, p->batch,
                    p->out_h, p->out_w, (long long)p->out_pixel_stride);
    return VIVIM_OK;
}

int vivim_head_concat_fwd(const vivim_head_concat_params* p, void* stream) {
    const char* fn = "head_concat_fwd";
    if (int rc = check_head_concat(p, fn, false)) return rc;
    if (!vivim::head_concat_dispatch(*p, false, as_stream(stream)))
        return fail(VIVIM_ERR_UNSUPPORTED, "%s not implemented for type %d", fn, p->itype);
    return after_launch(fn);
}

int vivim_head_concat_bwd(const vivim_head_concat_params* p, void* stream) {
    const char* fn = "head_concat_bwd";
    if (int rc = check_head_concat(p, fn, true)) return rc;
    if (!vivim::head_concat_dispatch(*p, true, as_stream(stream)))
        return fail(VIVIM_ERR_UNSUPPORTED, "%s not implemented for type %d", fn, p->itype);
    return after_launch(fn);
}


static int check_binary_metrics(const vivim_binary_metrics_params* p, const char* fn) {
    if (p == nullptr) return fail(VIVIM_ERR_INVALID, "%s: params is NULL", fn);
    if (int rc = check_struct_bytes(fn, "vivim_binary_metrics_params", p->struct_bytes, sizeof(*p))) return rc;
    if (!dtype_ok(p->ptype)) return fail(VIVIM_ERR_INVALID, "%s: ptype = %d: pred is fp32 / fp16 / bf16 (0 / 1 / 2)", fn, p->ptype);
    if (!dtype_ok(p->gtype) && p->gtype != 3)
        return fail(VIVIM_ERR_INVALID, "%s: gtype = %d: gt is fp32 / fp16 / bf16 (0 / 1 / 2) or uint8 / bool (3)", fn, p->gtype);
    if (p->batch <= 0 || p->height <= 0 || p->width <= 0)
        return fail(VIVIM_ERR_INVALID, "%s: batch = %d, height = %d, width = %d: every size must be positive", fn, p->batch, p->height, p->width);
    const int64_t pixels = (int64_t)p->height * p->width;
    if (pixels < 2) return fail(VIVIM_ERR_INVALID, "%s: height * width = %lld: the metrics need at least 2 pixels", fn, (long long)pixels);
    if (pixels > INT32_MAX - 4096 || (int64_t)p->batch * 32 > INT32_MAX)
        return fail(VIVIM_ERR_INVALID, "%s: batch = %d, height * width = %lld: the index range overflows int32", fn, p->batch, (long long)pixels);
    if (p->pred_batch_stride < pixels || p->gt_batch_stride < pixels)
        return fail(VIVIM_ERR_INVALID, "%s: pred_batch_stride = %lld, gt_batch_stride = %lld: an image has %lld elements", fn,
                    (long long)p->pred_batch_stride, (long long)p->gt_batch_stride, (long long)pixels);
    return VIVIM_OK;
}

size_t vivim_binary_metrics_workspace_bytes(const vivim_binary_metrics_params* p) {
    if (check_binary_metrics(p, "binary_metrics_workspace_bytes") != VIVIM_OK) return 0;
    return vivim::binary_metrics_workspace_bytes(*p);
}

int vivim_binary_metrics(const vivim_binary_metrics_params* p, void* stream) {
    const char* fn = "binary_metrics";
    if (int rc = check_binary_metrics(p, fn)) return rc;
    if (p->pred == nullptr || !aligned(p->pred, elem_bytes(p->ptype)))
        return fail(VIVIM_ERR_INVALID, "%s: pred at %p: need a %d-byte aligned pointer", fn, p->pred, elem_bytes(p->ptype));
    const int gbytes = p->gtype == 3 ? 1 : elem_bytes(p->gtype);
    if (p->gt == nullptr || !aligned(p->gt, gbytes))
        return fail(VIVIM_ERR_INVALID, "%s: gt at %p: need a %d-byte aligned pointer", fn, p->gt, gbytes);
    if (p->thresholds == nullptr || !aligned(p->thresholds, 4))
        return fail(VIVIM_ERR_INVALID, "%s: thresholds at %p: need 256 fp32 thresholds at a 4-byte aligned pointer", fn, p->thresholds);
    if (p->values == nullptr || !aligned(p->values, 8))
        return fail(VIVIM_ERR_INVALID, "%s: values at %p: need an 8-byte aligned pointer to (batch, 9) fp64", fn, p->values);
    if (p->hist != nullptr && !aligned(p->hist, 4))
        return fail(VIVIM_ERR_INVALID, "%s: hist at %p: need NULL or a 4-byte aligned pointer", fn, p->hist);
    if (p->state != nullptr && !aligned(p->state, 8))
        return fail(VIVIM_ERR_INVALID, "%s: state at %p: need NULL or an 8-byte aligned pointer to 10 fp64", fn, p->state);
    const size_t need = vivim::binary_metrics_workspace_bytes(*p);
    if (int rc = check_workspace(fn, "vivim_binary_metrics_workspace_bytes", p->workspace, p->workspace_bytes, 8, need)) return rc;
    if (!vivim::binary_metrics_dispatch(*p, as_stream(stream)))
        return fail(VIVIM_ERR_UNSUPPORTED, "%s not implemented for type %d", fn, p->ptype);
    return after_launch(fn);
}

}
```

vivim_amd/csrc/dwconv.hip:

```cpp
#include "ops.cuh"

namespace vivim {

constexpr int kDwTW = 4;
constexpr int kDwThreads = 256;

__device__ __forceinline__ float gelu_erf(float v) { return 0.5f * v * (1.0f + erff(v * 0.70710678118654752f)); }
__device__ __forceinline__ float gelu_erf_grad(float v) {
    return 0.5f * (1.0f + erff(v * 0.70710678118654752f)) + v * 0.39894228040143268f * __expf(-0.5f * v * v);
}

template <typename T, int KD, bool FLIP, int ACT = 0>
__global__ void __launch_bounds__(kDwThreads) dwconv_fwd_kernel(const vivim_dwconv_params p) {
    constexpr int CV = 16 / (int)sizeof(T);
    constexpr int CB = 8 * CV;
    constexpr int TAPS = KD * 9;
    constexpr int TW = kDwTW;
    __shared__ __attribute__((aligned(16))) float sw[TAPS * CB];
    const int tid = threadIdx.x;
    const int C = p.channels, D = p.depth, H = p.height, W = p.width;
    const int c0 = blockIdx.y * CB, b = blockIdx.z;
    const float* __restrict__ wt = static_cast<const float*>(p.wt);
    for (int i = tid; i < TAPS * CB; i += kDwThreads) {
        const int tap = i / CB, cc = i - tap * CB;
        sw[i] = (c0 + cc < C) ? wt[(int64_t)(FLIP ? TAPS - 1 - tap : tap) * C + c0 + cc] : 0.0f;
    }
    __syncthreads();
    const int cv = tid & 7, sp = tid >> 3;
    const int wtiles = (W + TW - 1) / TW;
    const int tile = blockIdx.x * (kDwThreads / 8) + sp;
    const int c = c0 + cv * CV;
    if (tile >= D * H * wtiles || c >= C) return;
    const int w0 = (tile % wtiles) * TW;
    const int h = (tile / wtiles) % H;
    const int d = tile / (wtiles * H);
    const T* __restrict__ x = static_cast<const T*>(p.x) + b * p.x_batch_stride + c;
    T* __restrict__ y = static_cast<T*>(p.y) + b * p.y_batch_stride + c;

    float acc[TW][CV];
#pragma unroll
    for (int j = 0; j < TW; ++j)
#pragma unroll
        for (int v = 0; v < CV; ++v) acc[j][v] = p.bias ? static_cast<const float*>(p.bias)[c + v] : 0.0f;
#pragma unroll
    for (int kd = 0; kd < KD; ++kd) {
        const int dd = d + kd - KD / 2;
        if (dd < 0 || dd >= D) continue;
#pragma unroll
        for (int kh = 0; kh < 3; ++kh) {
            const int hh = h + kh - 1;
            if (hh < 0 || hh >= H) continue;
            const int64_t row = ((int64_t)dd * H + hh) * W;
#pragma unroll
            for (int iw = -1; iw <= TW; ++iw) {
                const int ww = w0 + iw;
                float xv[CV];
                unpack(load_vec<T, CV>(x + (row + ww) * p.x_token_stride, ww >= 0 && ww < W), xv);
#pragma unroll
                for (int j = 0; j < TW; ++j) {
                    const int kw = iw - j + 1;
                    if (kw < 0 || kw > 2) continue;
                    const float* wp = sw + ((kd * 3 + kh) * 3 + kw) * CB + cv * CV;
#pragma unroll
                    for (int v = 0; v < CV; ++v) acc[j][v] = fmaf(wp[v], xv[v], acc[j][v]);
                }
            }
        }
    }
    const int64_t tok = ((int64_t)d * H + h) * W + w0;
    if (ACT == 1) {
#pragma unroll
        for (int j = 0; j < TW; ++j)
#pragma unroll
            for (int v = 0; v < CV; ++v) acc[j][v] = gelu_erf(acc[j][v]);
    } else if (ACT == 2) {
        const T* __restrict__ aux = static_cast<const T*>(p.aux) + b * p.aux_batch_stride + c;
#pragma unroll
        for (int j = 0; j < TW; ++j) {
            float gv[CV];
            unpack(load_vec<T, CV>(aux + (tok + j) * p.aux_token_stride, w0 + j < W), gv);
#pragma unroll
            for (int v = 0; v < CV; ++v) acc[j][v] = gv[v] * gelu_erf_grad(acc[j][v]);
        }
    }
#pragma unroll
    for (int j = 0; j < TW; ++j) store_vec<T, CV>(y + (tok + j) * p.y_token_stride, w0 + j < W, acc[j]);
}

template <typename T, int KD, bool DET = false>
__global__ void __launch_bounds__(kDwThreads) dwconv_wgrad_kernel(const vivim_dwconv_wgrad_params p, const int tiles_per_wave) {
    constexpr int CP = 2;
    constexpr int TAPS = KD * 9;
    constexpr int TW = kDwTW;
    __shared__ float red[(kDwThreads / kWave) * (TAPS + 1) * CP * kWave];
    const int tid = threadIdx.x, lane = tid & 63;
    const int wave = __builtin_amdgcn_readfirstlane(tid >> 6);
    const int C = p.channels, D = p.depth, H = p.height, W = p.width;
    const int c = blockIdx.y * (kWave * CP) + lane * CP, b = blockIdx.z;
    const bool cok = c < C;
    const T* __restrict__ x = static_cast<const T*>(p.x) + b * p.x_batch_stride + c;
    const T* __restrict__ dy = static_cast<const T*>(p.dy) + b * p.dy_batch_stride + c;
    const int wtiles = (W + TW - 1) / TW;
    const int ntiles = D * H * wtiles;
    const int t_lo = (blockIdx.x * (kDwThreads / kWave) + wave) * tiles_per_wave;
    const int t_hi = min(ntiles, t_lo + tiles_per_wave);

    float acc[TAPS][CP], db[CP] = {0.0f, 0.0f};
#pragma unroll
    for (int t = 0; t < TAPS; ++t) { acc[t][0] = 0.0f; acc[t][1] = 0.0f; }
    const T* __restrict__ safe_x = static_cast<const T*>(p.x) + b * p.x_batch_stride;
    const T* __restrict__ safe_dy = static_cast<const T*>(p.dy) + b * p.dy_batch_stride;
    for (int tile = t_lo; tile < t_hi; ++tile) {
        const int w0 = (tile % wtiles) * TW;
        const int h = (tile / wtiles) % H;
        const int d = tile / (wtiles * H);
        const int64_t tok = ((int64_t)d * H + h) * W + w0;
        RawK<T, CP> graw[TW], xraw[KD * 3][TW + 2];
#pragma unroll
        for (int j = 0; j < TW; ++j)
            graw[j] = load_vec_always<T, CP>(dy + (tok + j) * p.dy_token_stride, cok && w0 + j < W, safe_dy);
#pragma unroll
        for (int kd = 0; kd < KD; ++kd) {
            const int dd = d + kd - KD / 2;
#pragma unroll
            for (int kh = 0; kh < 3; ++kh) {
                const int hh = h + kh - 1;
                const bool rowok = cok && dd >= 0 && dd < D && hh >= 0 && hh < H;
                const int64_t row = ((int64_t)dd * H + hh) * W;
#pragma unroll
                for (int iw = -1; iw <= TW; ++iw) {
                    const int ww = w0 + iw;
                    xraw[kd * 3 + kh][iw + 1] = load_vec_always<T, CP>(x + (row + ww) * p.x_token_stride, rowok && ww >= 0 && ww < W, safe_x);
                }
            }
        }
        float g[TW][CP];
#pragma unroll
        for (int j = 0; j < TW; ++j) {
            unpack(graw[j], g[j]);
            db[0] += g[j][0];
            db[1] += g[j][1];
        }
#pragma unroll
        for (int r = 0; r < KD * 3; ++r) {
#pragma unroll
            for (int iw = -1; iw <= TW; ++iw) {
                float xv[CP];
                unpack(xraw[r][iw + 1], xv);
#pragma unroll
                for (int j = 0; j < TW; ++j) {
                    const int kw = iw - j + 1;
                    if (kw < 0 || kw > 2) continue;
                    const int tap = r * 3 + kw;
                    acc[tap][0] = fmaf(xv[0], g[j][0], acc[tap][0]);
                    acc[tap][1] = fmaf(xv[1], g[j][1], acc[tap][1]);
                }
            }
        }
    }
    float* mine = red + wave * (TAPS + 1) * CP * kWave;
#pragma unroll
    for (int t = 0; t < TAPS; ++t) {
        mine[(t * CP + 0) * kWave + lane] = acc[t][0];
        mine[(t * CP + 1) * kWave + lane] = acc[t][1];
    }
    mine[(TAPS * CP + 0) * kWave + lane] = db[0];
    mine[(TAPS * CP + 1) * kWave + lane] = db[1];
    __syncthreads();
    float* dwt = static_cast<float*>(p.dwt);
    for (int i = tid; i < (TAPS + 1) * CP * kWave; i += kDwThreads) {
        float s = 0.0f;
#pragma unroll
        for (int wv = 0; wv < kDwThreads / kWave; ++wv) s += red[wv * (TAPS + 1) * CP * kWave + i];
        const int ln = i & 63, cp = (i >> 6) & 1, t = i >> 7;
        const int cc = blockIdx.y * (kWave * CP) + ln * CP + cp;
        if (DET) {
            if (cc < C) dwt[((int64_t)blockIdx.z * gridDim.x + blockIdx.x) * (TAPS + 1) * C + (int64_t)t * C + cc] = s;
        } else if (cc < C) {
            if (t < TAPS) atomicAdd(dwt + (int64_t)t * C + cc, s);
            else if (p.dbias) atomicAdd(static_cast<float*>(p.dbias) + cc, s);
        }
    }
}

template <typename T>
static void dw_fwd(const vivim_dwconv_params& p, hipStream_t s) {
    constexpr int CV = 16 / (int)sizeof(T);
    const int wtiles = (p.width + kDwTW - 1) / kDwTW;
    const int ntiles = p.depth * p.height * wtiles;
    dim3 grid((ntiles + kDwThreads / 8 - 1) / (kDwThreads / 8), (p.channels + 8 * CV - 1) / (8 * CV), p.batch);
    if (p.act == 1 || p.act == 2) {
        if (p.kd == 3) {
            if (p.act == 1) hipLaunchKernelGGL((dwconv_fwd_kernel<T, 3, false, 1>), grid, dim3(kDwThreads), 0, s, p);
            else            hipLaunchKernelGGL((dwconv_fwd_kernel<T, 3, false, 2>), grid, dim3(kDwThreads), 0, s, p);
        } else {
            if (p.act == 1) hipLaunchKernelGGL((dwconv_fwd_kernel<T, 1, false, 1>), grid, dim3(kDwThreads), 0, s, p);
            else            hipLaunchKernelGGL((dwconv_fwd_kernel<T, 1, false, 2>), grid, dim3(kDwThreads), 0, s, p);
        }
        return;
    }
    if (p.kd == 3) {
        if (p.flip) hipLaunchKernelGGL((dwconv_fwd_kernel<T, 3, true>), grid, dim3(kDwThreads), 0, s, p);
        else        hipLaunchKernelGGL((dwconv_fwd_kernel<T, 3, false>), grid, dim3(kDwThreads), 0, s, p);
    } else {
        if (p.flip) hipLaunchKernelGGL((dwconv_fwd_kernel<T, 1, true>), grid, dim3(kDwThreads), 0, s, p);
        else        hipLaunchKernelGGL((dwconv_fwd_kernel<T, 1, false>), grid, dim3(kDwThreads), 0, s, p);
    }
}
static dim3 dw_wgrad_grid(const vivim_dwconv_wgrad_params& p, int& tpw_out) {
    const int wtiles = (p.width + kDwTW - 1) / kDwTW;
    const int ntiles = p.depth * p.height * wtiles;
    const int cgroups = (p.channels + 127) / 128;
    int blocks_x = (2048 + cgroups * p.batch - 1) / (cgroups * p.batch);
    int tpw = (ntiles + blocks_x * 4 - 1) / (blocks_x * 4);
    if (tpw < 8) tpw = 8;
    blocks_x = (ntiles + tpw * 4 - 1) / (tpw * 4);
    tpw_out = tpw;
    return dim3(blocks_x, cgroups, p.batch);
}
template <typename T, bool DET>
static void dw_wgrad(const vivim_dwconv_wgrad_params& p, hipStream_t s) {
    int tpw = 0;
    const dim3 grid = dw_wgrad_grid(p, tpw);
    if (p.kd == 3) hipLaunchKernelGGL((dwconv_wgrad_kernel<T, 3, DET>), grid, dim3(kDwThreads), 0, s, p, tpw);
    else           hipLaunchKernelGGL((dwconv_wgrad_kernel<T, 1, DET>), grid, dim3(kDwThreads), 0, s, p, tpw);
}

size_t dwconv_wgrad_det_workspace_bytes(const vivim_dwconv_wgrad_params& p) {
    int tpw = 0;
    const dim3 g = dw_wgrad_grid(p, tpw);
    return sizeof(float) * (size_t)g.x * g.z * (size_t)(p.kd * 9 + 1) * p.channels;
}
Launch dwconv_wgrad_det_dispatch(const vivim_dwconv_wgrad_params& p, void* ws, size_t bytes, hipStream_t s) {
    if (!det_ws_ok(ws, bytes, dwconv_wgrad_det_workspace_bytes(p))) return Launch::bad_workspace;
    vivim_dwconv_wgrad_params d = p;
    d.dwt = ws;
    if (!with_itype(p.itype, [&](auto t) { dw_wgrad<decltype(t), true>(d, s); })) return Launch::unsupported;
    int tpw = 0;
    const dim3 g = dw_wgrad_grid(p, tpw);
    const int taps = p.kd * 9, C = p.channels;
    const int64_t sstride = (int64_t)(taps + 1) * C;
    det_reduce(static_cast<const float*>(ws), (int)(g.x * g.z), det_out(static_cast<float*>(p.dwt), {taps, C}, {C, 1}), s, sstride);
    if (p.dbias)
        det_reduce(static_cast<const float*>(ws) + (int64_t)taps * C, (int)(g.x * g.z), det_out(static_cast<float*>(p.dbias), {C}, {1}), s, sstride);
    return Launch::ok;
}

bool dwconv_fwd_dispatch(const vivim_dwconv_params& p, hipStream_t s) {
    return with_itype(p.itype, [&](auto t) { dw_fwd<decltype(t)>(p, s); });
}
bool dwconv_wgrad_dispatch(const vivim_dwconv_wgrad_params& p, hipStream_t s) {
    return with_itype(p.itype, [&](auto t) { dw_wgrad<decltype(t), false>(p, s); });
}

}
```

vivim_amd/csrc/ops.cuh:

```cuda
#pragma once
#include "det.cuh"
#include "../../include/vivim_hip_ext.h"
#include "../../include/vivim_hip_ext_head.h"
#include "../../include/vivim_hip_ext_binary_metrics.h"

namespace vivim {

inline bool conv_channel_last(const vivim_conv_fwd_params& f) { return f.x_c_stride == 1 && f.x_l_stride > 1; }
bool conv_fwd_dispatch(const vivim_conv_fwd_params&, hipStream_t);
bool conv_bwd_dispatch(const vivim_conv_bwd_params&, hipStream_t);
size_t conv_bwd_det_workspace_bytes(const vivim_conv_fwd_params&);
Launch conv_bwd_det_dispatch(const vivim_conv_bwd_params&, void* ws, size_t bytes, hipStream_t);
bool conv_cl_fwd_dispatch(const vivim_conv_fwd_params&, hipStream_t);
bool conv_cl_bwd_dispatch(const vivim_conv_bwd_params&, hipStream_t);
size_t conv_cl_bwd_det_slots(const vivim_conv_fwd_params&);
bool conv_cl_bwd_det_launch(const vivim_conv_bwd_params&, hipStream_t);

bool ssm_fwd_dispatch(const vivim_ssm_fwd_params&, hipStream_t);
bool ssm_fwd_lean_dispatch(const vivim_ssm_fwd_params&, void* last_state, hipStream_t);
bool ssm_bwd_dispatch(const vivim_ssm_bwd_params&, hipStream_t);
Launch ssm_bwd_det_dispatch(const vivim_ssm_bwd_params&, void* det_ws, size_t det_ws_bytes, hipStream_t);
int scan_chunk_len(int itype);
int scan_ckpt_len(const vivim_ssm_fwd_params&);
size_t scan_fwd_workspace_bytes(const vivim_ssm_fwd_params&);
size_t scan_bwd_workspace_bytes(const vivim_ssm_fwd_params&);
size_t scan_bwd_det_workspace_bytes(const vivim_ssm_fwd_params&);
size_t scan_bwd_det_call_workspace_bytes(const vivim_ssm_bwd_params&);

void conv_update_launch(const vivim_conv_update_params&, hipStream_t);
void state_update_launch(const vivim_state_update_params&, hipStream_t);

bool dwconv_fwd_dispatch(const vivim_dwconv_params&, hipStream_t);
bool dwconv_wgrad_dispatch(const vivim_dwconv_wgrad_params&, hipStream_t);
size_t dwconv_wgrad_det_workspace_bytes(const vivim_dwconv_wgrad_params&);
Launch dwconv_wgrad_det_dispatch(const vivim_dwconv_wgrad_params&, void* ws, size_t bytes, hipStream_t);

template <bool GATHER> bool dir_dispatch(const vivim_dir_params&, hipStream_t);

bool layernorm_dispatch(const vivim_layernorm_params&, bool bwd, hipStream_t);
size_t layernorm_bwd_workspace_bytes(const vivim_layernorm_params&);
bool add_layernorm_dispatch(const vivim_add_layernorm_params&, bool bwd, hipStream_t);
size_t add_layernorm_bwd_workspace_bytes(const vivim_add_layernorm_params&);

bool token_layernorm_dispatch(const vivim_token_layernorm_params&, bool bwd, hipStream_t);
bool token_layernorm_pair_ok(int itype, int otype);
size_t token_layernorm_bwd_workspace_bytes(const vivim_token_layernorm_params&);
bool token_add_norm_dispatch(const vivim_token_add_norm_params&, bool bwd, hipStream_t);
bool token_add_norm_pair_ok(int btype, int rtype);
size_t token_add_norm_bwd_workspace_bytes(const vivim_token_add_norm_params&);

bool wgrad_nt_dispatch(const vivim_wgrad_nt_params&, hipStream_t);

bool seg_loss_dispatch(const vivim_seg_loss_params&, bool bwd, hipStream_t);
size_t seg_loss_workspace_bytes(const vivim_seg_loss_params&);
bool seg_metrics_dispatch(const vivim_seg_metrics_params&, hipStream_t);
size_t seg_metrics_workspace_bytes(const vivim_seg_metrics_params&);
bool structure_loss_dispatch(const vivim_structure_loss_params&, bool bwd, hipStream_t);
size_t structure_loss_workspace_bytes(const vivim_structure_loss_params&);
int64_t structure_loss_tiles(const vivim_structure_loss_params&);

bool upsample_dispatch(const vivim_upsample_params&, bool bwd, hipStream_t);
int64_t upsample_blocks(const vivim_upsample_params&, bool bwd);
bool decode_head_dispatch(const vivim_decode_head_params&, hipStream_t);
int64_t decode_head_blocks(const vivim_decode_head_params&);
int decode_head_max_hidden();

bool head_concat_dispatch(const vivim_head_concat_params&, bool bwd, hipStream_t);
int64_t head_concat_blocks(const vivim_head_concat_params&, bool bwd);

bool binary_metrics_dispatch(const vivim_binary_metrics_params&, hipStream_t);
size_t binary_metrics_workspace_bytes(const vivim_binary_metrics_params&);

void opt_grad_stats_launch(const vivim_opt_step_params&, hipStream_t);
void opt_finalise_launch(const vivim_opt_step_params&, hipStream_t);
void opt_adamw_launch(const vivim_opt_step_params&, hipStream_t);
void opt_grad_stats_mw_launch(const vivim_opt_step_params&, int dtype, hipStream_t);
void opt_adamw_mw_launch(const vivim_opt_step_params&, const void* masters, int dtype, hipStream_t);

}
```

vivim_amd/dirmap.py:

```python
import torch

from . import _lib
from ._lib import ITYPE


def _params(flat, stacked, nframes, csplit, scale, src, dst):
    B, C, L = flat.shape
    P = _lib.DirParams()
    P.batch, P.channels, P.seqlen, P.nframes, P.csplit, P.itype, P.scale = B, C, L, nframes, csplit, ITYPE[flat.dtype], scale
    P.flat_batch_stride, P.flat_c_stride = flat.stride(0), flat.stride(1)
    P.stk_batch_stride, P.stk_half_stride, P.stk_dir_stride, P.stk_c_stride = (stacked.stride(0), stacked.stride(1),
                                                                               stacked.stride(2), stacked.stride(3))
    P.src, P.dst = src.data_ptr(), dst.data_ptr()
    return P


def _scatter(flat, nframes, csplit, scale):
    if flat.stride(-1) != 1:
        flat = flat.contiguous()
    B, C, L = flat.shape
    stacked = _lib.empty((C // csplit, 3, csplit, B, L), flat.dtype, flat.device).permute(3, 0, 1, 2, 4)
    _lib.launch("vivim_dir_scatter", _params(flat, stacked, nframes, csplit, scale, flat, stacked), flat.device)
    return stacked


def _gather(stacked, nframes, scale, channel_major=False):
    if stacked.stride(-1) != 1:
        stacked = stacked.contiguous()
    B, H, _, csplit, L = stacked.shape
    if channel_major:
        flat = _lib.empty((H * csplit, B, L), stacked.dtype, stacked.device).permute(1, 0, 2)
    else:
        flat = _lib.empty((B, H * csplit, L), stacked.dtype, stacked.device)
    _lib.launch("vivim_dir_gather", _params(flat, stacked, nframes, csplit, scale, stacked, flat), stacked.device)
    return flat


class _StackFn(torch.autograd.Function):
    @staticmethod
    def forward(ctx, xz, nframes, halves):
        ctx.nframes = nframes
        return _scatter(xz, nframes, xz.shape[1] // halves, 1.0)

    @staticmethod
    def backward(ctx, g):
        return _gather(g, ctx.nframes, 1.0), None, None


class _CombineFn(torch.autograd.Function):
    @staticmethod
    def forward(ctx, o3, nframes):
        ctx.nframes = nframes
        B, _, D, L = o3.shape
        return _gather(o3.view(B, 1, 3, D, L), nframes, 1.0 / 3.0, channel_major=True)

    @staticmethod
    def backward(ctx, g):
        B, D, L = g.shape
        return _scatter(g, ctx.nframes, D, 1.0 / 3.0).view(B, 3, D, L), None


def stack_directions(xz, nframes, halves=2):
    return _StackFn.apply(xz, nframes, halves)


def combine_directions(o3, nframes):
    return _CombineFn.apply(o3, nframes)
```

vivim_amd/dwconv.py:

```python
import os

import torch

from . import _lib
from ._lib import ITYPE, ptr


def supported(x, weight):
    if os.environ.get("VIVIM_NO_DWCONV") or not (x.is_cuda and x.dim() == 3 and x.dtype in ITYPE and x.stride(2) == 1):
        return False
    cv = 16 // x.element_size()
    ks = tuple(weight.shape[2:])
    return (weight.shape[1] == 1 and ks in ((3, 3), (3, 3, 3)) and x.shape[2] % cv == 0
            and x.stride(1) % cv == 0 and x.stride(0) % cv == 0 and x.data_ptr() % 16 == 0)


def _taps(weight):
    C = weight.shape[0]
    return weight.detach().reshape(C, -1).t().contiguous().float()


def _aligned(t):
    cv = 16 // t.element_size()
    if t.stride(2) != 1 or t.data_ptr() % 16 or t.stride(1) % cv or t.stride(0) % cv:
        t = t.contiguous()
    return t


def _run_fwd(x, wt, bias, dims, flip, act=0, aux=None):
    B, L, C = x.shape
    D, H, W = dims
    y = _lib.empty((B, L, C), x.dtype, x.device)
    P = _lib.DwConvParams()
    P.batch, P.depth, P.height, P.width, P.channels = B, D, H, W, C
    P.kd, P.itype, P.flip = wt.shape[0] // 9, ITYPE[x.dtype], int(flip)
    P.x_batch_stride, P.x_token_stride = x.stride(0), x.stride(1)
    P.y_batch_stride, P.y_token_stride = y.stride(0), y.stride(1)
    P.x, P.wt, P.y = x.data_ptr(), wt.data_ptr(), y.data_ptr()
    P.bias = ptr(bias)
    P.act = act
    if aux is not None:
        P.aux, P.aux_batch_stride, P.aux_token_stride = aux.data_ptr(), aux.stride(0), aux.stride(1)
    _lib.launch("vivim_dwconv_fwd", P, x.device)
    return y


def _run_wgrad(x, dy, wt, dims, has_bias):
    B, L, C = x.shape
    D, H, W = dims
    acc = _lib.zeros(wt.shape[0] * C + C, x.device)
    P = _lib.DwConvWgradParams()
    P.batch, P.depth, P.height, P.width, P.channels = B, D, H, W, C
    P.kd, P.itype = wt.shape[0] // 9, ITYPE[x.dtype]
    P.x_batch_stride, P.x_token_stride = x.stride(0), x.stride(1)
    P.dy_batch_stride, P.dy_token_stride = dy.stride(0), dy.stride(1)
    P.x, P.dy, P.dwt = x.data_ptr(), dy.data_ptr(), acc.data_ptr()
    P.dbias = acc.data_ptr() + 4 * wt.shape[0] * C if has_bias else None
    if _lib.deterministic():
        nbytes, ws = _lib.workspace("vivim_dwconv_wgrad_det_workspace_bytes", P, x.device)
        _lib.launch("vivim_dwconv_wgrad_det", P, x.device, ptr(ws), nbytes)
    else:
        _lib.launch("vivim_dwconv_wgrad", P, x.device)
    return acc


class DepthwiseConvTokensFn(torch.autograd.Function):
    @staticmethod
    def forward(ctx, x, weight, bias, D, H, W):
        assert x.shape[1] == D * H * W, "token count must equal D*H*W"
        wt = _taps(weight)
        ctx.save_for_backward(x, wt)
        ctx.dims, ctx.wshape, ctx.wdtype = (D, H, W), weight.shape, weight.dtype
        ctx.has_bias = bias is not None
        ctx.bias_dtype = bias.dtype if bias is not None else None
        return _run_fwd(x, wt, bias.detach().float().contiguous() if bias is not None else None, (D, H, W), False)

    @staticmethod
    def backward(ctx, dy):
        x, wt = ctx.saved_tensors
        D, H, W = ctx.dims
        dy = _aligned(dy)
        dx = _run_fwd(dy, wt, None, (D, H, W), True) if ctx.needs_input_grad[0] else None
        C = x.shape[2]
        acc = _run_wgrad(x, dy, wt, (D, H, W), ctx.has_bias)
        dweight = acc[:wt.shape[0] * C].view(wt.shape[0], C).t().reshape(ctx.wshape).to(ctx.wdtype)
        dbias = acc[wt.shape[0] * C:].to(ctx.bias_dtype) if ctx.has_bias else None
        return dx, dweight, dbias, None, None, None


class DepthwiseConvGeluTokensFn(torch.autograd.Function):

    @staticmethod
    def forward(ctx, x, weight, bias, D, H, W):
        assert x.shape[1] == D * H * W, "token count must equal D*H*W"
        wt = _taps(weight)
        bf = bias.detach().float().contiguous() if bias is not None else None
        ctx.save_for_backward(x, wt, bf)
        ctx.dims, ctx.wshape, ctx.wdtype = (D, H, W), weight.shape, weight.dtype
        ctx.bias_dtype = bias.dtype if bias is not None else None
        return _run_fwd(x, wt, bf, (D, H, W), False, act=1)

    @staticmethod
    def backward(ctx, dy):
        x, wt, bf = ctx.saved_tensors
        dims = ctx.dims
        dpre = _run_fwd(x, wt, bf, dims, False, act=2, aux=_aligned(dy))
        dx = _run_fwd(dpre, wt, None, dims, True) if ctx.needs_input_grad[0] else None
        C = x.shape[2]
        acc = _run_wgrad(x, dpre, wt, dims, bf is not None)
        dweight = acc[:wt.shape[0] * C].view(wt.shape[0], C).t().reshape(ctx.wshape).to(ctx.wdtype)
        dbias = acc[wt.shape[0] * C:].to(ctx.bias_dtype) if bf is not None else None
        return dx, dweight, dbias, None, None, None


def depthwise_conv_tokens(x, weight, bias, D, H, W):
    return DepthwiseConvTokensFn.apply(x, weight, bias, D, H, W)


def depthwise_conv_gelu_tokens(x, weight, bias, D, H, W):
    return DepthwiseConvGeluTokensFn.apply(x, weight, bias, D, H, W)
```

vivim_amd/layernorm.py:

```python
import ctypes

import torch

from . import _lib
from ._lib import ITYPE, ptr


def supported(x, weight):
    if _lib.deterministic():
        return False
    if not (x.is_cuda and x.dim() == 3 and x.dtype in ITYPE and weight is not None and weight.dtype == torch.float32):
        return False
    B, L, C = x.shape
    e = 16 // x.element_size()
    return (x.stride(1) == 1 and C <= 512 and L % e == 0 and x.stride(0) % e == 0 and x.stride(2) % e == 0
            and x.data_ptr() % 16 == 0 and x.stride(2) >= L)


def worthwhile(x):
    return x.shape[0] * x.shape[1] >= 4096


def _params(x, out_dtype, eps):
    B, L, C = x.shape
    P = _lib.LayerNormParams()
    P.batch, P.seqlen, P.channels, P.itype, P.otype, P.eps = B, L, C, ITYPE[x.dtype], ITYPE[out_dtype], eps
    P.x_batch_stride, P.x_c_stride = x.stride(0), x.stride(2)
    P.x = x.data_ptr()
    return P


def _norm_forward(P, x, weight, bias, out_dtype):
    B, L, C = x.shape
    y = _lib.empty((B, L, C), out_dtype, x.device)
    stats = _lib.empty((2, B, L), torch.float32, x.device)
    P.y_batch_stride, P.y_token_stride = L * C, C
    P.weight, P.bias = weight.data_ptr(), ptr(bias)
    P.y, P.mean = y.data_ptr(), stats.data_ptr()
    P.rstd = P.mean + 4 * B * L
    return y, stats


def _norm_backward(P, query, dy, weight, stats, out_dtype, has_bias):
    B, L, C = P.batch, P.seqlen, P.channels
    P.weight, P.mean = weight.data_ptr(), stats.data_ptr()
    P.rstd = P.mean + 4 * B * L
    if dy is None:
        return None, None
    if dy.dtype != out_dtype:
        dy = dy.to(out_dtype)
    if dy.stride(2) != 1 or dy.stride(1) < C:
        dy = dy.contiguous()
    P.dy, P.y_batch_stride, P.y_token_stride = dy.data_ptr(), dy.stride(0), dy.stride(1)
    dwb = _lib.zeros(2 * C, stats.device)
    P.dweight = dwb.data_ptr()
    P.dbias = P.dweight + 4 * C if has_bias else None
    ws = _lib.workspace(query, P, stats.device)[1]
    P.workspace = ptr(ws)
    return dwb, (dy, ws)


class _LayerNormCM(torch.autograd.Function):
    @staticmethod
    def forward(ctx, x, weight, bias, eps, out_dtype):
        P = _params(x, out_dtype, eps)
        y, stats = _norm_forward(P, x, weight, bias, out_dtype)
        _lib.launch("vivim_layernorm_cm_fwd", P, x.device)
        ctx.save_for_backward(x, weight, stats)
        ctx.eps, ctx.has_bias, ctx.out_dtype = eps, bias is not None, out_dtype
        return y

    @staticmethod
    def backward(ctx, dy):
        x, weight, stats = ctx.saved_tensors
        B, L, C = x.shape
        dx = _lib.empty((B, C, L), x.dtype, x.device).transpose(1, 2)
        P = _params(x, ctx.out_dtype, ctx.eps)
        P.dx, P.dx_batch_stride, P.dx_c_stride = dx.data_ptr(), C * L, L
        dwb, _alive = _norm_backward(P, "vivim_layernorm_bwd_workspace_bytes", dy, weight, stats, ctx.out_dtype, ctx.has_bias)
        _lib.launch("vivim_layernorm_cm_bwd", P, x.device)
        return dx, dwb[:C], (dwb[C:] if ctx.has_bias else None), None, None


def layer_norm_cm(x, weight, bias, eps=1e-5, out_dtype=None):
    if out_dtype is None:
        out_dtype = torch.float32 if torch.is_autocast_enabled() else x.dtype
    return _LayerNormCM.apply(x, weight, bias, eps, out_dtype)


def _cm_ok(t, e):
    return (t.stride(1) == 1 and t.shape[1] % e == 0 and t.stride(0) % e == 0 and t.stride(2) % e == 0
            and t.data_ptr() % 16 == 0 and t.stride(2) >= t.shape[1])


def add_norm_supported(x, branch, weight=None):
    if _lib.deterministic():
        return False
    if not (x.is_cuda and x.dim() == 3 and x.dtype in ITYPE and branch.device == x.device and branch.shape == x.shape):
        return False
    if weight is not None and weight.dtype != torch.float32:
        return False
    if not (branch.dtype == x.dtype or (x.dtype == torch.float32 and branch.dtype in (torch.float16, torch.bfloat16))):
        return False
    C = x.shape[2]
    return C <= 512 and _cm_ok(x, 16 // x.element_size()) and branch.stride(2) == 1 and branch.stride(1) >= C


def _add_params(x, branch, scale):
    B, L, C = x.shape
    P = _lib.AddLayerNormParams()
    P.batch, P.seqlen, P.channels, P.itype, P.btype, P.otype = B, L, C, ITYPE[x.dtype], ITYPE[branch.dtype], ITYPE[x.dtype]
    P.scale = ptr(scale)
    return P


def _check_scale(scale, x):
    if scale is not None and not (scale.dtype == torch.float32 and scale.shape == (x.shape[0],) and scale.is_contiguous()
                                  and scale.device == x.device):
        raise ValueError("scale must be a contiguous (batch,) float32 tensor on x's device")


def _as_cm(g, like):
    if g.dtype != like.dtype:
        g = g.to(like.dtype)
    if not _cm_ok(g, 16 // g.element_size()):
        g = g.transpose(1, 2).contiguous().transpose(1, 2)
    return g


def _add_forward(x, branch, scale, P):
    B, L, C = x.shape
    x_new = _lib.empty((B, C, L), x.dtype, x.device).transpose(1, 2)
    P.x_batch_stride, P.x_c_stride = x.stride(0), x.stride(2)
    P.x_new_batch_stride, P.x_new_c_stride = C * L, L
    P.branch_batch_stride, P.branch_token_stride = branch.stride(0), branch.stride(1)
    P.x, P.branch, P.x_new = x.data_ptr(), branch.data_ptr(), x_new.data_ptr()
    return x_new


class _AddLayerNormCM(torch.autograd.Function):
    @staticmethod
    def forward(ctx, x, branch, weight, bias, scale, eps, out_dtype):
        P = _add_params(x, branch, scale)
        P.otype, P.eps = ITYPE[out_dtype], eps
        x_new = _add_forward(x, branch, scale, P)
        y, stats = _norm_forward(P, x, weight, bias, out_dtype)
        _lib.launch("vivim_add_layernorm_cm_fwd", P, x.device)
        ctx.save_for_backward(x_new, weight, stats, scale)
        ctx.eps, ctx.has_bias, ctx.out_dtype, ctx.branch_dtype = eps, bias is not None, out_dtype, branch.dtype
        ctx.set_materialize_grads(False)
        return x_new, y

    @staticmethod
    def backward(ctx, dres, dy):
        if dres is None and dy is None:
            return (None,) * 7
        x_new, weight, stats, scale = ctx.saved_tensors
        B, L, C = x_new.shape
        P = _lib.AddLayerNormParams()
        P.batch, P.seqlen, P.channels, P.eps = B, L, C, ctx.eps
        P.itype, P.btype, P.otype = ITYPE[x_new.dtype], ITYPE[ctx.branch_dtype], ITYPE[ctx.out_dtype]
        P.scale = ptr(scale)
        P.x_new_batch_stride, P.x_new_c_stride = x_new.stride(0), x_new.stride(2)
        P.x_new = x_new.data_ptr()
        dwb, _alive = _norm_backward(P, "vivim_add_layernorm_bwd_workspace_bytes", dy, weight, stats, ctx.out_dtype, ctx.has_bias)
        if dres is not None:
            dres = _as_cm(dres, x_new)
            P.dres, P.dres_batch_stride, P.dres_c_stride = dres.data_ptr(), dres.stride(0), dres.stride(2)
        dx = _lib.empty((B, C, L), x_new.dtype, x_new.device).transpose(1, 2)
        P.dx, P.dx_batch_stride, P.dx_c_stride = dx.data_ptr(), C * L, L
        dbranch = None
        if ctx.needs_input_grad[1]:
            dbranch = _lib.empty((B, L, C), ctx.branch_dtype, x_new.device)
            P.dbranch, P.dbranch_batch_stride, P.dbranch_token_stride = dbranch.data_ptr(), L * C, C
        _lib.launch("vivim_add_layernorm_cm_bwd", P, x_new.device)
        return (dx, dbranch, (dwb[:C] if dwb is not None else None),
                (dwb[C:] if dwb is not None and ctx.has_bias else None), None, None, None)


class _AddCM(torch.autograd.Function):
    @staticmethod
    def forward(ctx, x, branch, scale):
        P = _add_params(x, branch, scale)
        x_new = _add_forward(x, branch, scale, P)
        _lib.launch("vivim_add_layernorm_cm_fwd", P, x.device)
        ctx.save_for_backward(scale)
        ctx.branch_dtype = branch.dtype
        return x_new

    @staticmethod
    def backward(ctx, dres):
        scale, = ctx.saved_tensors
        if not ctx.needs_input_grad[1]:
            return dres, None, None
        dres = _as_cm(dres, dres)
        B, L, C = dres.shape
        dbranch = _lib.empty((B, L, C), ctx.branch_dtype, dres.device)
        P = _lib.AddLayerNormParams()
        P.batch, P.seqlen, P.channels = B, L, C
        P.itype, P.btype, P.otype = ITYPE[dres.dtype], ITYPE[ctx.branch_dtype], ITYPE[dres.dtype]
        P.scale = ptr(scale)
        P.dres, P.dres_batch_stride, P.dres_c_stride = dres.data_ptr(), dres.stride(0), dres.stride(2)
        P.dbranch, P.dbranch_batch_stride, P.dbranch_token_stride = dbranch.data_ptr(), L * C, C
        _lib.launch("vivim_add_layernorm_cm_bwd", P, dres.device)
        return dres, dbranch, None


def add_layer_norm_cm(x, branch, weight, bias, eps=1e-5, scale=None):
    _check_scale(scale, x)
    out_dtype = torch.float32 if torch.is_autocast_enabled() else x.dtype
    return _AddLayerNormCM.apply(x, branch, weight, bias, scale, eps, out_dtype)


def add_cm(x, branch, scale=None):
    _check_scale(scale, x)
    return _AddCM.apply(x, branch, scale)


TM_MAX_C = 1024


def _rows(x):
    if x.dim() == 0 or x.numel() == 0:
        return None
    C = x.shape[-1]
    if x.dim() == 1:
        return 1, C
    rows, stride = x.shape[-2], x.stride(-2)
    for d in range(x.dim() - 3, -1, -1):
        if x.shape[d] == 1:
            continue
        if rows == 1:
            stride = x.stride(d)
        elif x.stride(d) != stride * rows:
            return None
        rows *= x.shape[d]
    return (rows, stride) if rows > 1 else (1, C)


def tm_pair_ok(in_dtype, out_dtype):
    return in_dtype in ITYPE and out_dtype in ITYPE and (out_dtype == in_dtype or torch.float32 in (in_dtype, out_dtype))


def tm_rows(x, weight, bias=None):
    if not (x.is_cuda and x.dtype in ITYPE and x.dim() >= 1 and x.stride(-1) == 1 and 1 <= x.shape[-1] <= TM_MAX_C):
        return None
    if weight is None:
        return None
    for t in (weight, bias):
        if t is not None and not (t.dtype == torch.float32 and t.device == x.device and t.shape == (x.shape[-1],)
                                  and t.is_contiguous()):
            return None
    rs = _rows(x)
    return rs if rs is not None and rs[1] >= x.shape[-1] and rs[0] < 2 ** 31 else None


def tm_supported(x, weight, bias=None):
    return tm_rows(x, weight, bias) is not None


def tm_worthwhile(x):
    return x.numel() >= 1 << 21


def tm_workspace_slots(rows):
    return min(1024, (rows + 3) // 4)


class _LayerNormTM(torch.autograd.Function):
    @staticmethod
    def forward(ctx, x, weight, bias, eps, out_dtype, need_stats, rs):
        rows, C = rs[0], x.shape[-1]
        P = _lib.TokenLayerNormParams()
        P.struct_bytes = ctypes.sizeof(_lib.TokenLayerNormParams)
        P.rows, P.channels, P.itype, P.otype, P.eps = rows, C, ITYPE[x.dtype], ITYPE[out_dtype], eps
        P.x, P.x_row_stride = x.data_ptr(), rs[1]
        y = _lib.empty(tuple(x.shape), out_dtype, x.device)
        P.y, P.y_row_stride = y.data_ptr(), C
        P.weight, P.bias = weight.data_ptr(), ptr(bias)
        stats = None
        if need_stats:
            stats = _lib.empty((2, rows), torch.float32, x.device)
            P.mean = stats.data_ptr()
            P.rstd = P.mean + 4 * rows
        _lib.launch("vivim_token_layernorm_fwd", P, x.device)
        ctx.save_for_backward(x, weight, stats)
        ctx.P, ctx.has_bias, ctx.out_dtype = P, bias is not None, out_dtype
        return y

    @staticmethod
    def backward(ctx, dy):
        x, weight, stats = ctx.saved_tensors
        P, C = ctx.P, x.shape[-1]
        if dy.dtype != ctx.out_dtype:
            dy = dy.to(ctx.out_dtype)
        rs = _rows(dy) if dy.stride(-1) == 1 else None
        if rs is None or rs[1] < C:
            dy = dy.contiguous()
            rs = (P.rows, C)
        dx = _lib.empty(tuple(x.shape), x.dtype, x.device)
        P.dy, P.dy_row_stride, P.dx, P.dx_row_stride = dy.data_ptr(), rs[1], dx.data_ptr(), C
        need_w, need_b = ctx.needs_input_grad[1], ctx.has_bias and ctx.needs_input_grad[2]
        dwb = ws = None
        P.dweight = P.dbias = P.workspace = None
        if need_w or need_b:
            dwb = _lib.empty((2, C), torch.float32, x.device)
            P.dweight = dwb.data_ptr() if need_w else None
            P.dbias = dwb.data_ptr() + 4 * C if need_b else None
            ws = _lib.empty((tm_workspace_slots(P.rows) * 2 * C,), torch.float32, x.device)
            P.workspace = ws.data_ptr()
        _lib.launch("vivim_token_layernorm_bwd", P, x.device)
        return dx, (dwb[0] if need_w else None), (dwb[1] if need_b else None), None, None, None, None


def layer_norm_tm(x, weight, bias, eps=1e-5, out_dtype=None, rows=None):
    if out_dtype is None:
        out_dtype = torch.float32 if torch.is_autocast_enabled() else x.dtype
    if rows is None:
        rows = tm_rows(x, weight, bias)
        if rows is None:
            raise ValueError("layer_norm_tm: unsupported tensors (tm_supported)")
    if not tm_pair_ok(x.dtype, out_dtype):
        raise ValueError(f"layer_norm_tm: {x.dtype} rows with a {out_dtype} output are not built")
    need_stats = torch.is_grad_enabled() and (x.requires_grad or weight.requires_grad or (bias is not None and bias.requires_grad))
    return _LayerNormTM.apply(x, weight, bias, eps, out_dtype, need_stats, rows)


def tm_add_pair_ok(branch_dtype, res_dtype):
    return branch_dtype in ITYPE and (res_dtype == branch_dtype or res_dtype == torch.float32)


def tm_add_rows(res, branch, weight=None, bias=None):
    if not (res.is_cuda and branch.is_cuda and res.device == branch.device and tuple(res.shape) == tuple(branch.shape)):
        return None
    if not (res.dim() >= 1 and tm_add_pair_ok(branch.dtype, res.dtype) and 1 <= res.shape[-1] <= TM_MAX_C):
        return None
    if res.stride(-1) != 1 or branch.stride(-1) != 1:
        return None
    for t in (weight, bias):
        if t is not None and not (t.dtype == torch.float32 and t.device == res.device and tuple(t.shape) == (res.shape[-1],)
                                  and t.is_contiguous()):
            return None
    a, b = _rows(res), _rows(branch)
    if a is None or b is None or min(a[1], b[1]) < res.shape[-1] or a[0] >= 2 ** 31:
        return None
    return a[0], a[1], b[1]


def tm_add_supported(res, branch, weight=None, bias=None):
    return tm_add_rows(res, branch, weight, bias) is not None


def tm_add_worthwhile(res):
    return False


def _grad_rows(g, dtype, rows, C):
    if g.dtype != dtype:
        g = g.to(dtype)
    rs = _rows(g) if g.stride(-1) == 1 else None
    if rs is None or rs[1] < C:
        return g.contiguous(), C
    return g, rs[1]


def _add_norm_params(rows, C, branch_dtype, res_dtype, scale, eps=0.0, rms=False):
    P = _lib.TokenAddNormParams()
    P.struct_bytes = ctypes.sizeof(_lib.TokenAddNormParams)
    P.rows, P.channels, P.eps, P.rms = rows, C, eps, int(rms)
    P.btype = P.otype = ITYPE[branch_dtype]
    P.rtype = ITYPE[res_dtype]
    if scale is not None:
        P.scale, P.rows_per_sample = scale.data_ptr(), rows // scale.shape[0]
    return P


class _AddNormTM(torch.autograd.Function):

    @staticmethod
    def forward(ctx, res, branch, weight, bias, scale, eps, rms, need_stats, rows, res_dtype):
        n, res_stride, branch_stride = rows
        C = branch.shape[-1]
        P = _add_norm_params(n, C, branch.dtype, res_dtype or branch.dtype, scale, eps, rms)
        P.branch, P.branch_row_stride = branch.data_ptr(), branch_stride
        if res is not None:
            P.res, P.res_row_stride = res.data_ptr(), res_stride
        res_new = None
        if res_dtype is not None:
            res_new = _lib.empty(tuple(branch.shape), res_dtype, branch.device)
            P.res_out, P.res_out_row_stride = res_new.data_ptr(), C
        y = _lib.empty(tuple(branch.shape), branch.dtype, branch.device)
        P.y, P.y_row_stride = y.data_ptr(), C
        P.weight, P.bias = weight.data_ptr(), ptr(bias)
        stats = None
        if need_stats:
            stats = _lib.empty((2, n), torch.float32, branch.device)
            P.mean = stats.data_ptr()
            P.rstd = P.mean + 4 * n
        _lib.launch("vivim_token_add_norm_fwd", P, branch.device)
        ctx.save_for_backward(res_new if res_new is not None else branch, weight, stats, scale)
        ctx.h_stride = C if res_new is not None else branch_stride
        ctx.eps, ctx.rms, ctx.has_bias, ctx.branch_dtype, ctx.has_res = eps, rms, bias is not None, branch.dtype, res is not None
        ctx.set_materialize_grads(False)
        return res_new, y

    @staticmethod
    def backward(ctx, dres, dy):
        if dres is None and dy is None:
            return (None,) * 10
        h, weight, stats, scale = ctx.saved_tensors
        C, n = h.shape[-1], stats.shape[1]
        P = _add_norm_params(n, C, ctx.branch_dtype, h.dtype, scale, ctx.eps, ctx.rms)
        P.res_out, P.res_out_row_stride = h.data_ptr(), ctx.h_stride
        P.weight, P.mean = weight.data_ptr(), stats.data_ptr()
        P.rstd = P.mean + 4 * n
        if dy is not None:
            dy, P.dy_row_stride = _grad_rows(dy, ctx.branch_dtype, n, C)
            P.dy = dy.data_ptr()
        if dres is not None:
            dres, P.dres_row_stride = _grad_rows(dres, h.dtype, n, C)
            P.dres = dres.data_ptr()
        need_res, need_branch = ctx.has_res and ctx.needs_input_grad[0], ctx.needs_input_grad[1]
        shared = scale is None and ctx.branch_dtype == h.dtype and (need_res or need_branch)
        dres_in = dbranch = None
        if need_res or shared:
            dres_in = _lib.empty(tuple(h.shape), h.dtype, h.device)
            P.dres_in, P.dres_in_row_stride = dres_in.data_ptr(), C
        if need_branch and not shared:
            dbranch = _lib.empty(tuple(h.shape), ctx.branch_dtype, h.device)
            P.dbranch, P.dbranch_row_stride = dbranch.data_ptr(), C
        need_w = dy is not None and ctx.needs_input_grad[2]
        need_b = dy is not None and ctx.has_bias and ctx.needs_input_grad[3]
        dwb = ws = None
        if need_w or need_b:
            dwb = _lib.empty((2, C), torch.float32, h.device)
            P.dweight = dwb.data_ptr() if need_w else None
            P.dbias = dwb.data_ptr() + 4 * C if need_b else None
            ws = _lib.empty((tm_workspace_slots(n) * 2 * C,), torch.float32, h.device)
            P.workspace = ws.data_ptr()
        _lib.launch("vivim_token_add_norm_bwd", P, h.device)
        if shared:
            dbranch = dres_in if need_branch else None
            dres_in = dres_in if need_res else None
        return (dres_in, dbranch, (dwb[0] if need_w else None), (dwb[1] if need_b else None)) + (None,) * 6


class _AddTM(torch.autograd.Function):
    @staticmethod
    def forward(ctx, res, branch, scale, rows):
        n, res_stride, branch_stride = rows
        C = res.shape[-1]
        P = _add_norm_params(n, C, branch.dtype, res.dtype, scale)
        P.branch, P.branch_row_stride, P.res, P.res_row_stride = branch.data_ptr(), branch_stride, res.data_ptr(), res_stride
        res_new = _lib.empty(tuple(res.shape), res.dtype, res.device)
        P.res_out, P.res_out_row_stride = res_new.data_ptr(), C
        _lib.launch("vivim_token_add_norm_fwd", P, res.device)
        ctx.save_for_backward(scale)
        ctx.branch_dtype, ctx.n = branch.dtype, n
        return res_new

    @staticmethod
    def backward(ctx, dres):
        scale, = ctx.saved_tensors
        if not ctx.needs_input_grad[1]:
            return dres, None, None, None
        if scale is None and ctx.branch_dtype == dres.dtype:
            return dres, dres, None, None
        C = dres.shape[-1]
        g, stride = _grad_rows(dres, dres.dtype, ctx.n, C)
        P = _add_norm_params(ctx.n, C, ctx.branch_dtype, g.dtype, scale)
        P.dres, P.dres_row_stride = g.data_ptr(), stride
        dbranch = _lib.empty(tuple(g.shape), ctx.branch_dtype, g.device)
        P.dbranch, P.dbranch_row_stride = dbranch.data_ptr(), C
        _lib.launch("vivim_token_add_norm_bwd", P, g.device)
        return dres, dbranch, None, None


def _check_scale_tm(scale, res, rows):
    if scale is None:
        return
    if not (scale.dtype == torch.float32 and scale.dim() == 1 and scale.shape[0] == res.shape[0] and scale.is_contiguous()
            and scale.device == res.device and rows % scale.shape[0] == 0):
        raise ValueError("scale must be a contiguous (res.shape[0],) float32 tensor on res's device")


def _requires_grad(*ts):
    return torch.is_grad_enabled() and any(t is not None and t.requires_grad for t in ts)


def add_layer_norm_tm(res, branch, weight, bias, eps=1e-5, scale=None, out_dtype=None, rms=False, rows=None):
    if out_dtype is not None and out_dtype != branch.dtype:
        raise ValueError(f"add_layer_norm_tm: a {branch.dtype} branch with a {out_dtype} output is not built")
    if not tm_add_pair_ok(branch.dtype, res.dtype):
        raise ValueError(f"add_layer_norm_tm: a {branch.dtype} branch on a {res.dtype} residual is not built")
    if rows is None:
        rows = tm_add_rows(res, branch, weight, bias)
        if rows is None or weight is None:
            raise ValueError("add_layer_norm_tm: unsupported tensors (tm_add_supported)")
    _check_scale_tm(scale, res, rows[0])
    return _AddNormTM.apply(res, branch, weight, bias, scale, eps, rms, _requires_grad(res, branch, weight, bias), rows, res.dtype)


def add_tm(res, branch, scale=None, rows=None):
    if not tm_add_pair_ok(branch.dtype, res.dtype):
        raise ValueError(f"add_tm: a {branch.dtype} branch on a {res.dtype} residual is not built")
    if rows is None:
        rows = tm_add_rows(res, branch)
        if rows is None:
            raise ValueError("add_tm: unsupported tensors (tm_add_supported)")
    _check_scale_tm(scale, res, rows[0])
    return _AddTM.apply(res, branch, scale, rows)


def norm_tm_no_residual(x, weight, bias, eps, rms, res_dtype=None):
    rows = tm_add_rows(x, x, weight, bias)
    if rows is None or weight is None:
        raise ValueError("norm_tm_no_residual: unsupported tensors (tm_add_supported)")
    if res_dtype is not None and not tm_add_pair_ok(x.dtype, res_dtype):
        raise ValueError(f"norm_tm_no_residual: {x.dtype} rows with a {res_dtype} residual are not built")
    return _AddNormTM.apply(None, x, weight, bias, None, eps, rms, _requires_grad(x, weight, bias), rows, res_dtype)


def rms_norm_tm(x, weight, bias=None, eps=1e-5, out_dtype=None):
    if out_dtype is not None and out_dtype != x.dtype:
        raise ValueError(f"rms_norm_tm: {x.dtype} rows with a {out_dtype} output are not built")
    return norm_tm_no_residual(x, weight, bias, eps, True)[1]
```

Measured before the change: 218.9.

## Move dwconv, layernorm and direction autograd nodes into a C++ extension

Adds a pybind C++ extension that implements the depthwise-conv, channel-major layernorm and direction stack/combine autograd nodes natively, calling libvivim_hip directly instead of going through Python ctypes parameter filling. It also adds a module-layout dwconv entry point that reads and writes weights in the PyTorch (C, taps) layout, so the weight transposes and copies around it are no longer needed, with a zeroing kernel for the gradients. The aim is to cut per-call Python and launch overhead and the extra layout copies, at the cost of a new build artifact and duplicated logic between the Python and C++ paths.

After: 208.5. -4.7%, worse.

```diff
diff --git a/__graft_entry__.py b/__graft_entry__.py
--- a/__graft_entry__.py
+++ b/__graft_entry__.py
@@ -15,6 +15,7 @@
     import re
     header = open(os.path.join(ROOT, "include", "vivim_hip.h")).read()
     assert L.vivim_abi_version() == int(re.search(r"#define VIVIM_ABI_VERSION (\d+)", header).group(1))
+    _lib.nodes()
     import causal_conv1d
     import mamba_ssm
     import modeling.vivim
diff --git a/include/vivim_hip_ext_dwconv.h b/include/vivim_hip_ext_dwconv.h
--- /dev/null
+++ b/include/vivim_hip_ext_dwconv.h
@@ -0,0 +1,48 @@
+#ifndef VIVIM_HIP_EXT_DWCONV_H
+#define VIVIM_HIP_EXT_DWCONV_H
+
+#include "vivim_hip.h"
+
+#ifdef __cplusplus
+extern "C" {
+#endif
+
+typedef struct {
+    int32_t struct_bytes;
+    int32_t batch, depth, height, width, channels;
+    int32_t kd;
+    int32_t itype;
+    int32_t flip;
+    int32_t act;
+    int64_t x_batch_stride, x_token_stride;
+    int64_t y_batch_stride, y_token_stride;
+    int64_t aux_batch_stride, aux_token_stride;
+    const void *x;
+    const void *weight;
+    const void *bias;
+    const void *aux;
+    void *y;
+} vivim_dwconv_ml_params;
+
+typedef struct {
+    int32_t struct_bytes;
+    int32_t batch, depth, height, width, channels;
+    int32_t kd;
+    int32_t itype;
+    int64_t x_batch_stride, x_token_stride;
+    int64_t dy_batch_stride, dy_token_stride;
+    const void *x;
+    const void *dy;
+    void *dweight;
+    void *dbias;
+} vivim_dwconv_ml_wgrad_params;
+
+int vivim_dwconv_ml_fwd(const vivim_dwconv_ml_params *p, void *stream);
+int vivim_dwconv_ml_wgrad(const vivim_dwconv_ml_wgrad_params *p, void *stream);
+size_t vivim_dwconv_ml_wgrad_det_workspace_bytes(const vivim_dwconv_ml_wgrad_params *p);
+int vivim_dwconv_ml_wgrad_det(const vivim_dwconv_ml_wgrad_params *p, void *det_ws, size_t det_ws_bytes, void *stream);
+
+#ifdef __cplusplus
+}
+#endif
+#endif
diff --git a/vivim_amd/_lib.py b/vivim_amd/_lib.py
--- a/vivim_amd/_lib.py
+++ b/vivim_amd/_lib.py
@@ -1,8 +1,10 @@
 import collections
 import ctypes
+import importlib.util
 import os
 import re
 import subprocess
+import sys
 
 import torch
 
@@ -160,8 +162,48 @@
 def build(force=False):
     if force:
         subprocess.check_call(["make", "-C", CSRC, "clean"])
-    subprocess.check_call(["make", "-C", CSRC, "-j4"])
+    subprocess.check_call(["make", "-C", CSRC, "-j4", "PYTHON=" + sys.executable])
     return SO_PATH
+
+
+NODES_PATH = os.path.join(CSRC, "_vivim_nodes.so")
+_nodes = None
+_nodes_on = not os.environ.get("VIVIM_NO_NATIVE_NODES")
+
+
+def nodes():
+    global _nodes
+    if _nodes is None:
+        if os.environ.get("VIVIM_LIB"):
+            raise ImportError("the C++ nodes link csrc/libvivim_hip.so; VIVIM_LIB names another library")
+        if not os.path.exists(NODES_PATH):
+            raise ImportError(f"{NODES_PATH} is missing: run `make -C vivim_amd/csrc`")
+        lib()
+        spec = importlib.util.spec_from_file_location("_vivim_nodes", NODES_PATH)
+        mod = importlib.util.module_from_spec(spec)
+        spec.loader.exec_module(mod)
+        if mod.abi_version() != ABI_VERSION:
+            raise ImportError("_vivim_nodes.so was built against another libvivim_hip.so")
+        _nodes = mod
+    return _nodes
+
+
+def set_native_nodes(on):
+    global _nodes_on
+    prev, _nodes_on = _nodes_on, bool(on)
+    return prev
+
+
+def native_nodes():
+    if not _nodes_on or GUARD or (_profile is not None and _profile[1]):
+        return None
+    if _nodes is None:
+        try:
+            nodes()
+        except ImportError:
+            set_native_nodes(False)
+            return None
+    return _nodes
 
 
 def lib():
diff --git a/vivim_amd/csrc/capi.hip b/vivim_amd/csrc/capi.hip
--- a/vivim_amd/csrc/capi.hip
+++ b/vivim_amd/csrc/capi.hip
@@ -267,7 +267,7 @@
     return VIVIM_OK;
 }
 
-int vivim_dwconv_fwd(const vivim_dwconv_params* p, void* stream) {
+static int check_dw_fwd(const vivim_dwconv_params* p) {
     VCHECK(p != nullptr);
     if (int rc = check_dw_dims(p->batch, p->depth, p->height, p->width, p->channels, p->kd, p->itype)) return rc;
     VCHECK(p->x && p->wt && p->y);
@@ -279,6 +279,11 @@
     if (p->act == 2)
         VCHECK(p->aux && aligned16(p->aux) && p->aux_token_stride % cv == 0 &&
                p->aux_batch_stride % cv == 0);
+    return VIVIM_OK;
+}
+
+int vivim_dwconv_fwd(const vivim_dwconv_params* p, void* stream) {
+    if (int rc = check_dw_fwd(p)) return rc;
     if (!vivim::dwconv_fwd_dispatch(*p, as_stream(stream)))
         return fail(VIVIM_ERR_UNSUPPORTED, "dwconv_fwd not implemented for input type %d", p->itype);
     return after_launch("dwconv_fwd");
@@ -1023,4 +1028,83 @@
     return after_launch(fn);
 }
 
-}
+static vivim_dwconv_wgrad_params dw_ml_wgrad_params(const vivim_dwconv_ml_wgrad_params* p) {
+    vivim_dwconv_wgrad_params q;
+    memset(&q, 0, sizeof(q));
+    q.batch = p->batch, q.depth = p->depth, q.height = p->height, q.width = p->width, q.channels = p->channels;
+    q.kd = p->kd, q.itype = p->itype;
+    q.x_batch_stride = p->x_batch_stride, q.x_token_stride = p->x_token_stride;
+    q.dy_batch_stride = p->dy_batch_stride, q.dy_token_stride = p->dy_token_stride;
+    q.x = p->x, q.dy = p->dy, q.dwt = p->dweight, q.dbias = p->dbias;
+    return q;
+}
+
+static int check_dw_ml_wgrad(const vivim_dwconv_ml_wgrad_params* p, const char* fn, vivim_dwconv_wgrad_params* q) {
+    VCHECK(p != nullptr);
+    if (int rc = check_struct_bytes(fn, "vivim_dwconv_ml_wgrad_params", p->struct_bytes, sizeof(*p))) return rc;
+    *q = dw_ml_wgrad_params(p);
+    if (int rc = check_dw_wgrad(q)) return rc;
+    VCHECK(aligned(p->dweight, 4) && aligned(p->dbias, 4));
+    return VIVIM_OK;
+}
+
+static int zero_dw_ml_grads(const vivim_dwconv_ml_wgrad_params* p, const char* fn, hipStream_t s) {
+    const int64_t wn = (int64_t)p->kd * 9 * p->channels, bn = p->channels;
+    VCHECK(wn + bn <= INT32_MAX);
+    float* dw = static_cast<float*>(p->dweight);
+    const bool joined = p->dbias == dw + wn;
+    vivim::dwconv_zero(dw, joined ? wn + bn : wn, s);
+    if (p->dbias && !joined) vivim::dwconv_zero(static_cast<float*>(p->dbias), bn, s);
+    return after_launch(fn);
+}
+
+int vivim_dwconv_ml_fwd(const vivim_dwconv_ml_params* p, void* stream) {
+    const char* fn = "dwconv_ml_fwd";
+    VCHECK(p != nullptr);
+    if (int rc = check_struct_bytes(fn, "vivim_dwconv_ml_params", p->struct_bytes, sizeof(*p))) return rc;
+    vivim_dwconv_params q;
+    memset(&q, 0, sizeof(q));
+    q.batch = p->batch, q.depth = p->depth, q.height = p->height, q.width = p->width, q.channels = p->channels;
+    q.kd = p->kd, q.itype = p->itype, q.flip = p->flip, q.act = p->act;
+    q.x_batch_stride = p->x_batch_stride, q.x_token_stride = p->x_token_stride;
+    q.y_batch_stride = p->y_batch_stride, q.y_token_stride = p->y_token_stride;
+    q.aux_batch_stride = p->aux_batch_stride, q.aux_token_stride = p->aux_token_stride;
+    q.x = p->x, q.wt = p->weight, q.bias = p->bias, q.aux = p->aux, q.y = p->y;
+    if (int rc = check_dw_fwd(&q)) return rc;
+    VCHECK(aligned(p->weight, 4));
+    if (!vivim::dwconv_fwd_dispatch(q, as_stream(stream), true))
+        return fail(VIVIM_ERR_UNSUPPORTED, "%s not implemented for input type %d", fn, p->itype);
+    return after_launch(fn);
+}
+
+int vivim_dwconv_ml_wgrad(const vivim_dwconv_ml_wgrad_params* p, void* stream) {
+    const char* fn = "dwconv_ml_wgrad";
+    vivim_dwconv_wgrad_params q;
+    if (int rc = check_dw_ml_wgrad(p, fn, &q)) return rc;
+    if (int rc = zero_dw_ml_grads(p, fn, as_stream(stream))) return rc;
+    if (!vivim::dwconv_wgrad_dispatch(q, as_stream(stream), true))
+        return fail(VIVIM_ERR_UNSUPPORTED, "%s not implemented for input type %d", fn, p->itype);
+    return after_launch(fn);
+}
+
+size_t vivim_dwconv_ml_wgrad_det_workspace_bytes(const vivim_dwconv_ml_wgrad_params* p) {
+    if (!p || p->struct_bytes != (int32_t)sizeof(*p)) return 0;
+    const vivim_dwconv_wgrad_params q = dw_ml_wgrad_params(p);
+    return vivim_dwconv_wgrad_det_workspace_bytes(&q);
+}
+
+int vivim_dwconv_ml_wgrad_det(const vivim_dwconv_ml_wgrad_params* p, void* det_ws, size_t det_ws_bytes, void* stream) {
+    const char* fn = "dwconv_ml_wgrad_det";
+    vivim_dwconv_wgrad_params q;
+    if (int rc = check_dw_ml_wgrad(p, fn, &q)) return rc;
+    const size_t need = vivim::dwconv_wgrad_det_workspace_bytes(q);
+    if (!vivim::det_ws_ok(det_ws, det_ws_bytes, need))
+        return bad_workspace(fn, "vivim_dwconv_ml_wgrad_det_workspace_bytes", det_ws_bytes, det_ws, 16, need);
+    if (!dtype_ok(p->itype)) return fail(VIVIM_ERR_UNSUPPORTED, "%s not implemented for input type %d", fn, p->itype);
+    if (int rc = zero_dw_ml_grads(p, fn, as_stream(stream))) return rc;
+    if (vivim::dwconv_wgrad_det_dispatch(q, det_ws, det_ws_bytes, as_stream(stream), true) != Launch::ok)
+        return fail(VIVIM_ERR_UNSUPPORTED, "%s not implemented for input type %d", fn, p->itype);
+    return after_launch(fn);
+}
+
+}
diff --git a/vivim_amd/csrc/dwconv.hip b/vivim_amd/csrc/dwconv.hip
--- a/vivim_amd/csrc/dwconv.hip
+++ b/vivim_amd/csrc/dwconv.hip
@@ -10,8 +10,13 @@
     return 0.5f * (1.0f + erff(v * 0.70710678118654752f)) + v * 0.39894228040143268f * __expf(-0.5f * v * v);
 }
 
+struct DwTapLayout { int tap, chan; };
+static DwTapLayout dw_tap_layout(bool module_layout, int kd, int channels) {
+    return module_layout ? DwTapLayout{1, kd * 9} : DwTapLayout{channels, 1};
+}
+
 template <typename T, int KD, bool FLIP, int ACT = 0>
-__global__ void __launch_bounds__(kDwThreads) dwconv_fwd_kernel(const vivim_dwconv_params p) {
+__global__ void __launch_bounds__(kDwThreads) dwconv_fwd_kernel(const vivim_dwconv_params p, const DwTapLayout wl) {
     constexpr int CV = 16 / (int)sizeof(T);
     constexpr int CB = 8 * CV;
     constexpr int TAPS = KD * 9;
@@ -23,7 +28,7 @@
     const float* __restrict__ wt = static_cast<const float*>(p.wt);
     for (int i = tid; i < TAPS * CB; i += kDwThreads) {
         const int tap = i / CB, cc = i - tap * CB;
-        sw[i] = (c0 + cc < C) ? wt[(int64_t)(FLIP ? TAPS - 1 - tap : tap) * C + c0 + cc] : 0.0f;
+        sw[i] = (c0 + cc < C) ? wt[(int64_t)(FLIP ? TAPS - 1 - tap : tap) * wl.tap + (int64_t)(c0 + cc) * wl.chan] : 0.0f;
     }
     __syncthreads();
     const int cv = tid & 7, sp = tid >> 3;
@@ -88,7 +93,8 @@
 }
 
 template <typename T, int KD, bool DET = false>
-__global__ void __launch_bounds__(kDwThreads) dwconv_wgrad_kernel(const vivim_dwconv_wgrad_params p, const int tiles_per_wave) {
+__global__ void __launch_bounds__(kDwThreads) dwconv_wgrad_kernel(const vivim_dwconv_wgrad_params p, const int tiles_per_wave,
+                                                                  const DwTapLayout wl) {
     constexpr int CP = 2;
     constexpr int TAPS = KD * 9;
     constexpr int TW = kDwTW;
@@ -168,6 +174,25 @@
     mine[(TAPS * CP + 1) * kWave + lane] = db[1];
     __syncthreads();
     float* dwt = static_cast<float*>(p.dwt);
+    if (!DET && wl.tap == 1) {
+        const int cbase = blockIdx.y * (kWave * CP);
+        for (int j = tid; j < TAPS * CP * kWave; j += kDwThreads) {
+            const int cl = j / TAPS, t = j - cl * TAPS;
+            const int i = (t * CP + (cl & 1)) * kWave + (cl >> 1);
+            float s = 0.0f;
+#pragma unroll
+            for (int wv = 0; wv < kDwThreads / kWave; ++wv) s += red[wv * (TAPS + 1) * CP * kWave + i];
+            if (cbase + cl < C) atomicAdd(dwt + (int64_t)cbase * TAPS + j, s);
+        }
+        if (p.dbias && tid < CP * kWave) {
+            const int i = (TAPS * CP + (tid & 1)) * kWave + (tid >> 1);
+            float s = 0.0f;
+#pragma unroll
+            for (int wv = 0; wv < kDwThreads / kWave; ++wv) s += red[wv * (TAPS + 1) * CP * kWave + i];
+            if (cbase + tid < C) atomicAdd(static_cast<float*>(p.dbias) + cbase + tid, s);
+        }
+        return;
+    }
     for (int i = tid; i < (TAPS + 1) * CP * kWave; i += kDwThreads) {
         float s = 0.0f;
 #pragma unroll
@@ -177,34 +202,44 @@
         if (DET) {
             if (cc < C) dwt[((int64_t)blockIdx.z * gridDim.x + blockIdx.x) * (TAPS + 1) * C + (int64_t)t * C + cc] = s;
         } else if (cc < C) {
-            if (t < TAPS) atomicAdd(dwt + (int64_t)t * C + cc, s);
+            if (t < TAPS) atomicAdd(dwt + (int64_t)t * wl.tap + (int64_t)cc * wl.chan, s);
             else if (p.dbias) atomicAdd(static_cast<float*>(p.dbias) + cc, s);
         }
     }
 }
 
+__global__ void __launch_bounds__(256) dwconv_zero_kernel(float* __restrict__ out, const int n) {
+    for (int i = blockIdx.x * 256 + threadIdx.x; i < n; i += gridDim.x * 256) out[i] = 0.0f;
+}
+void dwconv_zero(float* out, int64_t n, hipStream_t s) {
+    if (n <= 0) return;
+    const int blocks = (int)std::min<int64_t>((n + 255) / 256, 256);
+    hipLaunchKernelGGL(dwconv_zero_kernel, dim3(blocks), dim3(256), 0, s, out, (int)n);
+}
+
 template <typename T>
-static void dw_fwd(const vivim_dwconv_params& p, hipStream_t s) {
+static void dw_fwd(const vivim_dwconv_params& p, bool module_layout, hipStream_t s) {
+    const DwTapLayout wl = dw_tap_layout(module_layout, p.kd, p.channels);
     constexpr int CV = 16 / (int)sizeof(T);
     const int wtiles = (p.width + kDwTW - 1) / kDwTW;
     const int ntiles = p.depth * p.height * wtiles;
     dim3 grid((ntiles + kDwThreads / 8 - 1) / (kDwThreads / 8), (p.channels + 8 * CV - 1) / (8 * CV), p.batch);
     if (p.act == 1 || p.act == 2) {
         if (p.kd == 3) {
-            if (p.act == 1) hipLaunchKernelGGL((dwconv_fwd_kernel<T, 3, false, 1>), grid, dim3(kDwThreads), 0, s, p);
-            else            hipLaunchKernelGGL((dwconv_fwd_kernel<T, 3, false, 2>), grid, dim3(kDwThreads), 0, s, p);
+            if (p.act == 1) hipLaunchKernelGGL((dwconv_fwd_kernel<T, 3, false, 1>), grid, dim3(kDwThreads), 0, s, p, wl);
+            else            hipLaunchKernelGGL((dwconv_fwd_kernel<T, 3, false, 2>), grid, dim3(kDwThreads), 0, s, p, wl);
         } else {
-            if (p.act == 1) hipLaunchKernelGGL((dwconv_fwd_kernel<T, 1, false, 1>), grid, dim3(kDwThreads), 0, s, p);
-            else            hipLaunchKernelGGL((dwconv_fwd_kernel<T, 1, false, 2>), grid, dim3(kDwThreads), 0, s, p);
+            if (p.act == 1) hipLaunchKernelGGL((dwconv_fwd_kernel<T, 1, false, 1>), grid, dim3(kDwThreads), 0, s, p, wl);
+            else            hipLaunchKernelGGL((dwconv_fwd_kernel<T, 1, false, 2>), grid, dim3(kDwThreads), 0, s, p, wl);
         }
         return;
     }
     if (p.kd == 3) {
-        if (p.flip) hipLaunchKernelGGL((dwconv_fwd_kernel<T, 3, true>), grid, dim3(kDwThreads), 0, s, p);
-        else        hipLaunchKernelGGL((dwconv_fwd_kernel<T, 3, false>), grid, dim3(kDwThreads), 0, s, p);
+        if (p.flip) hipLaunchKernelGGL((dwconv_fwd_kernel<T, 3, true>), grid, dim3(kDwThreads), 0, s, p, wl);
+        else        hipLaunchKernelGGL((dwconv_fwd_kernel<T, 3, false>), grid, dim3(kDwThreads), 0, s, p, wl);
     } else {
-        if (p.flip) hipLaunchKernelGGL((dwconv_fwd_kernel<T, 1, true>), grid, dim3(kDwThreads), 0, s, p);
-        else        hipLaunchKernelGGL((dwconv_fwd_kernel<T, 1, false>), grid, dim3(kDwThreads), 0, s, p);
+        if (p.flip) hipLaunchKernelGGL((dwconv_fwd_kernel<T, 1, true>), grid, dim3(kDwThreads), 0, s, p, wl);
+        else        hipLaunchKernelGGL((dwconv_fwd_kernel<T, 1, false>), grid, dim3(kDwThreads), 0, s, p, wl);
     }
 }
 static dim3 dw_wgrad_grid(const vivim_dwconv_wgrad_params& p, int& tpw_out) {
@@ -219,11 +254,12 @@
     return dim3(blocks_x, cgroups, p.batch);
 }
 template <typename T, bool DET>
-static void dw_wgrad(const vivim_dwconv_wgrad_params& p, hipStream_t s) {
+static void dw_wgrad(const vivim_dwconv_wgrad_params& p, bool module_layout, hipStream_t s) {
+    const DwTapLayout wl = dw_tap_layout(module_layout, p.kd, p.channels);
     int tpw = 0;
     const dim3 grid = dw_wgrad_grid(p, tpw);
-    if (p.kd == 3) hipLaunchKernelGGL((dwconv_wgrad_kernel<T, 3, DET>), grid, dim3(kDwThreads), 0, s, p, tpw);
-    else           hipLaunchKernelGGL((dwconv_wgrad_kernel<T, 1, DET>), grid, dim3(kDwThreads), 0, s, p, tpw);
+    if (p.kd == 3) hipLaunchKernelGGL((dwconv_wgrad_kernel<T, 3, DET>), grid, dim3(kDwThreads), 0, s, p, tpw, wl);
+    else           hipLaunchKernelGGL((dwconv_wgrad_kernel<T, 1, DET>), grid, dim3(kDwThreads), 0, s, p, tpw, wl);
 }
 
 size_t dwconv_wgrad_det_workspace_bytes(const vivim_dwconv_wgrad_params& p) {
@@ -231,26 +267,27 @@
     const dim3 g = dw_wgrad_grid(p, tpw);
     return sizeof(float) * (size_t)g.x * g.z * (size_t)(p.kd * 9 + 1) * p.channels;
 }
-Launch dwconv_wgrad_det_dispatch(const vivim_dwconv_wgrad_params& p, void* ws, size_t bytes, hipStream_t s) {
+Launch dwconv_wgrad_det_dispatch(const vivim_dwconv_wgrad_params& p, void* ws, size_t bytes, hipStream_t s, bool module_layout) {
     if (!det_ws_ok(ws, bytes, dwconv_wgrad_det_workspace_bytes(p))) return Launch::bad_workspace;
     vivim_dwconv_wgrad_params d = p;
     d.dwt = ws;
-    if (!with_itype(p.itype, [&](auto t) { dw_wgrad<decltype(t), true>(d, s); })) return Launch::unsupported;
+    if (!with_itype(p.itype, [&](auto t) { dw_wgrad<decltype(t), true>(d, false, s); })) return Launch::unsupported;
     int tpw = 0;
     const dim3 g = dw_wgrad_grid(p, tpw);
     const int taps = p.kd * 9, C = p.channels;
     const int64_t sstride = (int64_t)(taps + 1) * C;
-    det_reduce(static_cast<const float*>(ws), (int)(g.x * g.z), det_out(static_cast<float*>(p.dwt), {taps, C}, {C, 1}), s, sstride);
+    const DwTapLayout wl = dw_tap_layout(module_layout, p.kd, C);
+    det_reduce(static_cast<const float*>(ws), (int)(g.x * g.z), det_out(static_cast<float*>(p.dwt), {taps, C}, {wl.tap, wl.chan}), s, sstride);
     if (p.dbias)
         det_reduce(static_cast<const float*>(ws) + (int64_t)taps * C, (int)(g.x * g.z), det_out(static_cast<float*>(p.dbias), {C}, {1}), s, sstride);
     return Launch::ok;
 }
 
-bool dwconv_fwd_dispatch(const vivim_dwconv_params& p, hipStream_t s) {
-    return with_itype(p.itype, [&](auto t) { dw_fwd<decltype(t)>(p, s); });
-}
-bool dwconv_wgrad_dispatch(const vivim_dwconv_wgrad_params& p, hipStream_t s) {
-    return with_itype(p.itype, [&](auto t) { dw_wgrad<decltype(t), false>(p, s); });
-}
-
-}
+bool dwconv_fwd_dispatch(const vivim_dwconv_params& p, hipStream_t s, bool module_layout) {
+    return with_itype(p.itype, [&](auto t) { dw_fwd<decltype(t)>(p, module_layout, s); });
+}
+bool dwconv_wgrad_dispatch(const vivim_dwconv_wgrad_params& p, hipStream_t s, bool module_layout) {
+    return with_itype(p.itype, [&](auto t) { dw_wgrad<decltype(t), false>(p, module_layout, s); });
+}
+
+}
diff --git a/vivim_amd/csrc/nodes.cpp b/vivim_amd/csrc/nodes.cpp
--- /dev/null
+++ b/vivim_amd/csrc/nodes.cpp
@@ -0,0 +1,361 @@
+#include <torch/extension.h>
+#include <ATen/Context.h>
+#include <c10/hip/HIPFunctions.h>
+#include <c10/hip/HIPGuard.h>
+#include <c10/hip/HIPStream.h>
+
+#include <cstring>
+#include <stdexcept>
+#include <string>
+
+#include "../../include/vivim_hip.h"
+#include "../../include/vivim_hip_ext_dwconv.h"
+
+namespace {
+
+using at::Tensor;
+using torch::autograd::AutogradContext;
+using torch::autograd::variable_list;
+using OptTensor = c10::optional<Tensor>;
+
+int itype_of(at::ScalarType t) {
+    switch (t) {
+        case at::kFloat: return VIVIM_F32;
+        case at::kHalf: return VIVIM_F16;
+        case at::kBFloat16: return VIVIM_BF16;
+        default: TORCH_CHECK(false, "vivim native node: dtype ", t, " is not one of float32, float16, bfloat16");
+    }
+}
+
+at::ScalarType dtype_of(int64_t itype) {
+    switch (itype) {
+        case VIVIM_F32: return at::kFloat;
+        case VIVIM_F16: return at::kHalf;
+        case VIVIM_BF16: return at::kBFloat16;
+        default: TORCH_CHECK(false, "vivim native node: unknown vivim_dtype_t ", itype);
+    }
+}
+
+const void* ptr(const OptTensor& t) { return t.has_value() && t->defined() ? t->data_ptr() : nullptr; }
+
+template <class F>
+void launch(const Tensor& t, F&& fn) {
+    TORCH_CHECK(t.is_cuda(), "vivim native node: expected a tensor on the GPU, got one on ", t.device());
+    const c10::DeviceIndex index = t.get_device();
+    c10::hip::OptionalHIPGuard guard;
+    if (index != c10::hip::current_device()) guard.set_index(index);
+    void* stream = c10::hip::getCurrentHIPStream(index).stream();
+    if (fn(stream) != VIVIM_OK) throw std::runtime_error(vivim_last_error());
+}
+
+bool deterministic() { return at::globalContext().deterministicAlgorithms(); }
+
+template <class P>
+pybind11::bytes bytes_of(const P& p) { return pybind11::bytes(reinterpret_cast<const char*>(&p), sizeof(P)); }
+
+
+Tensor dw_aligned(const Tensor& t) {
+    const int64_t cv = 16 / t.element_size();
+    if (t.stride(2) != 1 || reinterpret_cast<uintptr_t>(t.data_ptr()) % 16 || t.stride(1) % cv || t.stride(0) % cv) return t.contiguous();
+    return t;
+}
+
+Tensor dw_weight(const Tensor& weight) {
+    TORCH_CHECK(weight.dim() == 4 || weight.dim() == 5, "depthwise conv: weight must be (C, 1, 3, 3) or (C, 1, 3, 3, 3)");
+    return weight.detach().to(at::kFloat).contiguous();
+}
+
+struct DwFwd {
+    vivim_dwconv_ml_params P;
+    Tensor y;
+};
+
+DwFwd dw_fwd_fill(const Tensor& x, const Tensor& w32, const OptTensor& bias, int64_t D, int64_t H, int64_t W, int act, int flip,
+                  const OptTensor& aux) {
+    TORCH_CHECK(x.dim() == 3, "depthwise conv: x must be (B, D*H*W, C)");
+    DwFwd c;
+    c.y = at::empty({x.size(0), x.size(1), x.size(2)}, x.options());
+    vivim_dwconv_ml_params& P = c.P;
+    std::memset(&P, 0, sizeof(P));
+    P.struct_bytes = (int32_t)sizeof(P);
+    P.batch = (int32_t)x.size(0), P.depth = (int32_t)D, P.height = (int32_t)H, P.width = (int32_t)W, P.channels = (int32_t)x.size(2);
+    P.kd = w32.dim() == 5 ? 3 : 1, P.itype = itype_of(x.scalar_type()), P.flip = flip, P.act = act;
+    P.x_batch_stride = x.stride(0), P.x_token_stride = x.stride(1);
+    P.y_batch_stride = c.y.stride(0), P.y_token_stride = c.y.stride(1);
+    P.x = x.data_ptr(), P.weight = w32.data_ptr(), P.bias = ptr(bias), P.y = c.y.data_ptr();
+    if (aux.has_value()) P.aux = aux->data_ptr(), P.aux_batch_stride = aux->stride(0), P.aux_token_stride = aux->stride(1);
+    return c;
+}
+
+Tensor dw_fwd(const Tensor& x, const Tensor& w32, const OptTensor& bias, int64_t D, int64_t H, int64_t W, int act, int flip,
+              const OptTensor& aux = c10::nullopt) {
+    DwFwd c = dw_fwd_fill(x, w32, bias, D, H, W, act, flip, aux);
+    launch(x, [&](void* s) { return vivim_dwconv_ml_fwd(&c.P, s); });
+    return c.y;
+}
+
+struct DwWgrad {
+    vivim_dwconv_ml_wgrad_params P;
+    Tensor acc;
+};
+
+DwWgrad dw_wgrad_fill(const Tensor& x, const Tensor& dy, int64_t kd, int64_t D, int64_t H, int64_t W, bool has_bias) {
+    DwWgrad c;
+    const int64_t C = x.size(2), taps = kd * 9;
+    c.acc = at::empty({taps * C + C}, x.options().dtype(at::kFloat));
+    vivim_dwconv_ml_wgrad_params& P = c.P;
+    std::memset(&P, 0, sizeof(P));
+    P.struct_bytes = (int32_t)sizeof(P);
+    P.batch = (int32_t)x.size(0), P.depth = (int32_t)D, P.height = (int32_t)H, P.width = (int32_t)W, P.channels = (int32_t)C;
+    P.kd = (int32_t)kd, P.itype = itype_of(x.scalar_type());
+    P.x_batch_stride = x.stride(0), P.x_token_stride = x.stride(1);
+    P.dy_batch_stride = dy.stride(0), P.dy_token_stride = dy.stride(1);
+    P.x = x.data_ptr(), P.dy = dy.data_ptr(), P.dweight = c.acc.data_ptr();
+    P.dbias = has_bias ? static_cast<float*>(c.acc.data_ptr()) + taps * C : nullptr;
+    return c;
+}
+
+std::pair<Tensor, Tensor> dw_wgrad(const Tensor& x, const Tensor& dy, const Tensor& w32, at::IntArrayRef wshape, at::ScalarType wdtype,
+                                   int64_t D, int64_t H, int64_t W, bool has_bias, at::ScalarType bias_dtype) {
+    const int64_t C = x.size(2), kd = w32.dim() == 5 ? 3 : 1, taps = kd * 9;
+    DwWgrad c = dw_wgrad_fill(x, dy, kd, D, H, W, has_bias);
+    if (deterministic()) {
+        const size_t n = vivim_dwconv_ml_wgrad_det_workspace_bytes(&c.P);
+        Tensor ws = at::empty({(int64_t)n}, x.options().dtype(at::kByte));
+        launch(x, [&](void* s) { return vivim_dwconv_ml_wgrad_det(&c.P, n ? ws.data_ptr() : nullptr, n, s); });
+    } else {
+        launch(x, [&](void* s) { return vivim_dwconv_ml_wgrad(&c.P, s); });
+    }
+    Tensor dweight = c.acc.narrow(0, 0, taps * C).view(wshape).to(wdtype);
+    Tensor dbias = has_bias ? c.acc.narrow(0, taps * C, C).to(bias_dtype) : Tensor();
+    return {dweight, dbias};
+}
+
+struct DepthwiseConvTokens : public torch::autograd::Function<DepthwiseConvTokens> {
+    static Tensor forward(AutogradContext* ctx, const Tensor& x, const Tensor& weight, const OptTensor& bias, int64_t D, int64_t H,
+                          int64_t W, bool gelu) {
+        TORCH_CHECK(x.dim() == 3 && x.size(1) == D * H * W, "token count must equal D*H*W");
+        const bool has_bias = bias.has_value() && bias->defined();
+        Tensor w32 = dw_weight(weight);
+        OptTensor bf = has_bias ? OptTensor(bias->detach().to(at::kFloat).contiguous()) : c10::nullopt;
+        if (gelu && has_bias) ctx->save_for_backward({x, w32, *bf});
+        else ctx->save_for_backward({x, w32});
+        ctx->saved_data["dims"] = std::vector<int64_t>{D, H, W};
+        ctx->saved_data["wshape"] = weight.sizes().vec();
+        ctx->saved_data["wdtype"] = (int64_t)weight.scalar_type();
+        ctx->saved_data["has_bias"] = has_bias;
+        ctx->saved_data["bias_dtype"] = (int64_t)(has_bias ? bias->scalar_type() : at::kFloat);
+        ctx->saved_data["gelu"] = gelu;
+        return dw_fwd(x, w32, bf, D, H, W, gelu ? 1 : 0, 0);
+    }
+
+    static variable_list backward(AutogradContext* ctx, variable_list grads) {
+        const variable_list saved = ctx->get_saved_variables();
+        const Tensor &x = saved[0], &w32 = saved[1];
+        const std::vector<int64_t> dims = ctx->saved_data["dims"].toIntVector(), wshape = ctx->saved_data["wshape"].toIntVector();
+        const int64_t D = dims[0], H = dims[1], W = dims[2];
+        const bool has_bias = ctx->saved_data["has_bias"].toBool(), gelu = ctx->saved_data["gelu"].toBool();
+        Tensor dy = dw_aligned(grads[0]);
+        if (gelu)
+            dy = dw_fwd(x, w32, has_bias ? OptTensor(saved[2]) : c10::nullopt, D, H, W, 2, 0, dy);
+        Tensor dx = ctx->needs_input_grad(0) ? dw_fwd(dy, w32, c10::nullopt, D, H, W, 0, 1) : Tensor();
+        auto [dweight, dbias] = dw_wgrad(x, dy, w32, wshape, (at::ScalarType)ctx->saved_data["wdtype"].toInt(), D, H, W, has_bias,
+                                         (at::ScalarType)ctx->saved_data["bias_dtype"].toInt());
+        return {dx, dweight, dbias, Tensor(), Tensor(), Tensor(), Tensor()};
+    }
+};
+
+Tensor depthwise_conv_tokens(const Tensor& x, const Tensor& weight, const OptTensor& bias, int64_t D, int64_t H, int64_t W, bool gelu) {
+    return DepthwiseConvTokens::apply(x, weight, bias, D, H, W, gelu);
+}
+
+
+vivim_layernorm_params ln_params(const Tensor& x, at::ScalarType out_dtype, double eps) {
+    TORCH_CHECK(x.dim() == 3, "layer_norm_cm: x must be a (B, L, C) view");
+    vivim_layernorm_params P;
+    std::memset(&P, 0, sizeof(P));
+    P.batch = (int32_t)x.size(0), P.seqlen = (int32_t)x.size(1), P.channels = (int32_t)x.size(2);
+    P.itype = itype_of(x.scalar_type()), P.otype = itype_of(out_dtype), P.eps = (float)eps;
+    P.x_batch_stride = x.stride(0), P.x_c_stride = x.stride(2);
+    P.x = x.data_ptr();
+    return P;
+}
+
+struct LnFwd {
+    vivim_layernorm_params P;
+    Tensor y, stats;
+};
+
+LnFwd ln_fwd_fill(const Tensor& x, const Tensor& weight, const OptTensor& bias, double eps, at::ScalarType out_dtype) {
+    LnFwd c;
+    c.P = ln_params(x, out_dtype, eps);
+    const int64_t B = x.size(0), L = x.size(1), C = x.size(2);
+    c.y = at::empty({B, L, C}, x.options().dtype(out_dtype));
+    c.stats = at::empty({2, B, L}, x.options().dtype(at::kFloat));
+    c.P.y_batch_stride = L * C, c.P.y_token_stride = C;
+    c.P.weight = weight.data_ptr(), c.P.bias = ptr(bias);
+    c.P.y = c.y.data_ptr(), c.P.mean = c.stats.data_ptr();
+    c.P.rstd = static_cast<float*>(c.stats.data_ptr()) + B * L;
+    return c;
+}
+
+struct LnBwd {
+    vivim_layernorm_params P;
+    Tensor dx, dwb, dy, ws;
+};
+
+LnBwd ln_bwd_fill(const Tensor& x, const Tensor& weight, const Tensor& stats, const Tensor& dy_in, double eps, at::ScalarType out_dtype,
+                  bool has_bias) {
+    LnBwd c;
+    c.P = ln_params(x, out_dtype, eps);
+    const int64_t B = x.size(0), L = x.size(1), C = x.size(2);
+    c.dx = at::empty({B, C, L}, x.options()).transpose(1, 2);
+    c.P.dx = c.dx.data_ptr(), c.P.dx_batch_stride = C * L, c.P.dx_c_stride = L;
+    c.P.weight = weight.data_ptr(), c.P.mean = stats.data_ptr();
+    c.P.rstd = static_cast<float*>(stats.data_ptr()) + B * L;
+    c.dy = dy_in.scalar_type() == out_dtype ? dy_in : dy_in.to(out_dtype);
+    if (c.dy.stride(2) != 1 || c.dy.stride(1) < C) c.dy = c.dy.contiguous();
+    c.P.dy = c.dy.data_ptr(), c.P.y_batch_stride = c.dy.stride(0), c.P.y_token_stride = c.dy.stride(1);
+    c.dwb = at::zeros({2 * C}, stats.options());
+    c.P.dweight = c.dwb.data_ptr();
+    c.P.dbias = has_bias ? static_cast<float*>(c.dwb.data_ptr()) + C : nullptr;
+    const size_t n = vivim_layernorm_bwd_workspace_bytes(&c.P);
+    if (n) {
+        c.ws = at::empty({(int64_t)n}, stats.options().dtype(at::kByte));
+        c.P.workspace = c.ws.data_ptr();
+    }
+    return c;
+}
+
+std::tuple<Tensor, Tensor> layer_norm_cm_fwd(const Tensor& x, const Tensor& weight, const OptTensor& bias, double eps, int64_t otype) {
+    LnFwd c = ln_fwd_fill(x, weight, bias, eps, dtype_of(otype));
+    launch(x, [&](void* s) { return vivim_layernorm_cm_fwd(&c.P, s); });
+    return {c.y, c.stats};
+}
+
+std::tuple<Tensor, Tensor> layer_norm_cm_bwd(const Tensor& x, const Tensor& weight, const Tensor& stats, const Tensor& dy, double eps,
+                                             int64_t otype, bool has_bias) {
+    LnBwd c = ln_bwd_fill(x, weight, stats, dy, eps, dtype_of(otype), has_bias);
+    launch(x, [&](void* s) { return vivim_layernorm_cm_bwd(&c.P, s); });
+    return {c.dx, c.dwb};
+}
+
+
+vivim_dir_params dir_params(const Tensor& flat, const Tensor& stacked, int64_t nframes, int64_t csplit, double scale, const Tensor& src,
+                            const Tensor& dst) {
+    vivim_dir_params P;
+    std::memset(&P, 0, sizeof(P));
+    P.batch = (int32_t)flat.size(0), P.channels = (int32_t)flat.size(1), P.seqlen = (int32_t)flat.size(2);
+    P.nframes = (int32_t)nframes, P.csplit = (int32_t)csplit, P.itype = itype_of(flat.scalar_type()), P.scale = (float)scale;
+    P.flat_batch_stride = flat.stride(0), P.flat_c_stride = flat.stride(1);
+    P.stk_batch_stride = stacked.stride(0), P.stk_half_stride = stacked.stride(1);
+    P.stk_dir_stride = stacked.stride(2), P.stk_c_stride = stacked.stride(3);
+    P.src = src.data_ptr(), P.dst = dst.data_ptr();
+    return P;
+}
+
+struct DirCall {
+    vivim_dir_params P;
+    Tensor in, out;
+};
+
+DirCall scatter_fill(const Tensor& flat_in, int64_t nframes, int64_t csplit, double scale) {
+    TORCH_CHECK(flat_in.dim() == 3 && csplit > 0, "stack_directions: expected a (B, C, L) tensor");
+    DirCall c;
+    c.in = flat_in.stride(-1) != 1 ? flat_in.contiguous() : flat_in;
+    const int64_t B = c.in.size(0), C = c.in.size(1), L = c.in.size(2);
+    c.out = at::empty({C / csplit, 3, csplit, B, L}, c.in.options()).permute({3, 0, 1, 2, 4});
+    c.P = dir_params(c.in, c.out, nframes, csplit, scale, c.in, c.out);
+    return c;
+}
+
+DirCall gather_fill(const Tensor& stacked_in, int64_t nframes, double scale, bool channel_major) {
+    TORCH_CHECK(stacked_in.dim() == 5, "combine_directions: expected a (B, H, 3, csplit, L) tensor");
+    DirCall c;
+    c.in = stacked_in.stride(-1) != 1 ? stacked_in.contiguous() : stacked_in;
+    const int64_t B = c.in.size(0), Hh = c.in.size(1), csplit = c.in.size(3), L = c.in.size(4);
+    c.out = channel_major ? at::empty({Hh * csplit, B, L}, c.in.options()).permute({1, 0, 2}) : at::empty({B, Hh * csplit, L}, c.in.options());
+    c.P = dir_params(c.out, c.in, nframes, csplit, scale, c.in, c.out);
+    return c;
+}
+
+Tensor scatter(const Tensor& flat, int64_t nframes, int64_t csplit, double scale) {
+    DirCall c = scatter_fill(flat, nframes, csplit, scale);
+    launch(c.in, [&](void* s) { return vivim_dir_scatter(&c.P, s); });
+    return c.out;
+}
+
+Tensor gather(const Tensor& stacked, int64_t nframes, double scale, bool channel_major) {
+    DirCall c = gather_fill(stacked, nframes, scale, channel_major);
+    launch(c.in, [&](void* s) { return vivim_dir_gather(&c.P, s); });
+    return c.out;
+}
+
+struct StackDirections : public torch::autograd::Function<StackDirections> {
+    static Tensor forward(AutogradContext* ctx, const Tensor& xz, int64_t nframes, int64_t halves) {
+        ctx->saved_data["nframes"] = nframes;
+        return scatter(xz, nframes, xz.size(1) / halves, 1.0);
+    }
+    static variable_list backward(AutogradContext* ctx, variable_list grads) {
+        return {gather(grads[0], ctx->saved_data["nframes"].toInt(), 1.0, false), Tensor(), Tensor()};
+    }
+};
+
+struct CombineDirections : public torch::autograd::Function<CombineDirections> {
+    static Tensor forward(AutogradContext* ctx, const Tensor& o3, int64_t nframes) {
+        TORCH_CHECK(o3.dim() == 4 && o3.size(1) == 3, "combine_directions: expected a (B, 3, D, L) tensor");
+        ctx->saved_data["nframes"] = nframes;
+        return gather(o3.view({o3.size(0), 1, 3, o3.size(2), o3.size(3)}), nframes, 1.0 / 3.0, true);
+    }
+    static variable_list backward(AutogradContext* ctx, variable_list grads) {
+        const Tensor& g = grads[0];
+        const int64_t B = g.size(0), D = g.size(1), L = g.size(2);
+        return {scatter(g, ctx->saved_data["nframes"].toInt(), D, 1.0 / 3.0).view({B, 3, D, L}), Tensor()};
+    }
+};
+
+Tensor stack_directions(const Tensor& xz, int64_t nframes, int64_t halves) { return StackDirections::apply(xz, nframes, halves); }
+Tensor combine_directions(const Tensor& o3, int64_t nframes) { return CombineDirections::apply(o3, nframes); }
+
+
+pybind11::bytes dwconv_fwd_params(const Tensor& x, const Tensor& weight, const OptTensor& bias, int64_t D, int64_t H, int64_t W, int64_t act,
+                                  int64_t flip, const OptTensor& aux) {
+    return bytes_of(dw_fwd_fill(x, weight, bias, D, H, W, (int)act, (int)flip, aux).P);
+}
+pybind11::bytes dwconv_wgrad_params(const Tensor& x, const Tensor& dy, int64_t kd, int64_t D, int64_t H, int64_t W, bool has_bias) {
+    return bytes_of(dw_wgrad_fill(x, dy, kd, D, H, W, has_bias).P);
+}
+pybind11::bytes layernorm_fwd_params(const Tensor& x, const Tensor& weight, const OptTensor& bias, double eps, int64_t otype) {
+    return bytes_of(ln_fwd_fill(x, weight, bias, eps, dtype_of(otype)).P);
+}
+pybind11::bytes layernorm_bwd_params(const Tensor& x, const Tensor& weight, const Tensor& stats, const Tensor& dy, double eps, int64_t otype,
+                                     bool has_bias) {
+    return bytes_of(ln_bwd_fill(x, weight, stats, dy, eps, dtype_of(otype), has_bias).P);
+}
+pybind11::bytes dir_scatter_params(const Tensor& flat, int64_t nframes, int64_t csplit, double scale) {
+    return bytes_of(scatter_fill(flat, nframes, csplit, scale).P);
+}
+pybind11::bytes dir_gather_params(const Tensor& stacked, int64_t nframes, double scale, bool channel_major) {
+    return bytes_of(gather_fill(stacked, nframes, scale, channel_major).P);
+}
+
+}
+
+PYBIND11_MODULE(_vivim_nodes, m) {
+    m.doc() = "C++ autograd nodes over libvivim_hip.so (vivim_amd/csrc/nodes.cpp)";
+    namespace py = pybind11;
+    m.def("abi_version", [] { return vivim_abi_version(); });
+    m.def("depthwise_conv_tokens", &depthwise_conv_tokens, py::arg("x"), py::arg("weight"), py::arg("bias"), py::arg("D"), py::arg("H"),
+          py::arg("W"), py::arg("gelu"));
+    m.def("layer_norm_cm_fwd", &layer_norm_cm_fwd, py::arg("x"), py::arg("weight"), py::arg("bias"), py::arg("eps"), py::arg("otype"));
+    m.def("layer_norm_cm_bwd", &layer_norm_cm_bwd, py::arg("x"), py::arg("weight"), py::arg("stats"), py::arg("dy"), py::arg("eps"),
+          py::arg("otype"), py::arg("has_bias"));
+    m.def("stack_directions", &stack_directions, py::arg("xz"), py::arg("nframes"), py::arg("halves"));
+    m.def("combine_directions", &combine_directions, py::arg("o3"), py::arg("nframes"));
+    m.def("dwconv_fwd_params", &dwconv_fwd_params);
+    m.def("dwconv_wgrad_params", &dwconv_wgrad_params);
+    m.def("layernorm_fwd_params", &layernorm_fwd_params);
+    m.def("layernorm_bwd_params", &layernorm_bwd_params);
+    m.def("dir_scatter_params", &dir_scatter_params);
+    m.def("dir_gather_params", &dir_gather_params);
+}
diff --git a/vivim_amd/csrc/ops.cuh b/vivim_amd/csrc/ops.cuh
--- a/vivim_amd/csrc/ops.cuh
+++ b/vivim_amd/csrc/ops.cuh
@@ -3,6 +3,7 @@
 #include "../../include/vivim_hip_ext.h"
 #include "../../include/vivim_hip_ext_head.h"
 #include "../../include/vivim_hip_ext_binary_metrics.h"
+#include "../../include/vivim_hip_ext_dwconv.h"
 
 namespace vivim {
 
@@ -30,10 +31,11 @@
 void conv_update_launch(const vivim_conv_update_params&, hipStream_t);
 void state_update_launch(const vivim_state_update_params&, hipStream_t);
 
-bool dwconv_fwd_dispatch(const vivim_dwconv_params&, hipStream_t);
-bool dwconv_wgrad_dispatch(const vivim_dwconv_wgrad_params&, hipStream_t);
+bool dwconv_fwd_dispatch(const vivim_dwconv_params&, hipStream_t, bool module_layout = false);
+bool dwconv_wgrad_dispatch(const vivim_dwconv_wgrad_params&, hipStream_t, bool module_layout = false);
+void dwconv_zero(float* out, int64_t n, hipStream_t);
 size_t dwconv_wgrad_det_workspace_bytes(const vivim_dwconv_wgrad_params&);
-Launch dwconv_wgrad_det_dispatch(const vivim_dwconv_wgrad_params&, void* ws, size_t bytes, hipStream_t);
+Launch dwconv_wgrad_det_dispatch(const vivim_dwconv_wgrad_params&, void* ws, size_t bytes, hipStream_t, bool module_layout = false);
 
 template <bool GATHER> bool dir_dispatch(const vivim_dir_params&, hipStream_t);
 
diff --git a/vivim_amd/dirmap.py b/vivim_amd/dirmap.py
--- a/vivim_amd/dirmap.py
+++ b/vivim_amd/dirmap.py
@@ -61,8 +61,14 @@
 
 
 def stack_directions(xz, nframes, halves=2):
+    native = _lib.native_nodes()
+    if native is not None:
+        return native.stack_directions(xz, nframes, halves)
     return _StackFn.apply(xz, nframes, halves)
 
 
 def combine_directions(o3, nframes):
+    native = _lib.native_nodes()
+    if native is not None:
+        return native.combine_directions(o3, nframes)
     return _CombineFn.apply(o3, nframes)
diff --git a/vivim_amd/dwconv.py b/vivim_amd/dwconv.py
--- a/vivim_amd/dwconv.py
+++ b/vivim_amd/dwconv.py
@@ -4,6 +4,12 @@
 
 from . import _lib
 from ._lib import ITYPE, ptr
+
+
+ML_HEADER = os.path.join(os.path.dirname(_lib.HEADER), "vivim_hip_ext_dwconv.h")
+ML_STRUCT_NAMES = {"vivim_dwconv_ml_params": "DwConvMlParams", "vivim_dwconv_ml_wgrad_params": "DwConvMlWgradParams"}
+_, _classes, ML_ENTRY_POINTS = _lib.parse_header(_lib._read_header(ML_HEADER), ML_STRUCT_NAMES)
+DwConvMlParams, DwConvMlWgradParams = _classes["DwConvMlParams"], _classes["DwConvMlWgradParams"]
 
 
 def supported(x, weight):
@@ -114,8 +120,14 @@
 
 
 def depthwise_conv_tokens(x, weight, bias, D, H, W):
+    native = _lib.native_nodes()
+    if native is not None:
+        return native.depthwise_conv_tokens(x, weight, bias, D, H, W, False)
     return DepthwiseConvTokensFn.apply(x, weight, bias, D, H, W)
 
 
 def depthwise_conv_gelu_tokens(x, weight, bias, D, H, W):
+    native = _lib.native_nodes()
+    if native is not None:
+        return native.depthwise_conv_tokens(x, weight, bias, D, H, W, True)
     return DepthwiseConvGeluTokensFn.apply(x, weight, bias, D, H, W)
diff --git a/vivim_amd/layernorm.py b/vivim_amd/layernorm.py
--- a/vivim_amd/layernorm.py
+++ b/vivim_amd/layernorm.py
@@ -63,9 +63,13 @@
 class _LayerNormCM(torch.autograd.Function):
     @staticmethod
     def forward(ctx, x, weight, bias, eps, out_dtype):
-        P = _params(x, out_dtype, eps)
-        y, stats = _norm_forward(P, x, weight, bias, out_dtype)
-        _lib.launch("vivim_layernorm_cm_fwd", P, x.device)
+        native = _lib.native_nodes()
+        if native is not None:
+            y, stats = native.layer_norm_cm_fwd(x, weight, bias, eps, ITYPE[out_dtype])
+        else:
+            P = _params(x, out_dtype, eps)
+            y, stats = _norm_forward(P, x, weight, bias, out_dtype)
+            _lib.launch("vivim_layernorm_cm_fwd", P, x.device)
         ctx.save_for_backward(x, weight, stats)
         ctx.eps, ctx.has_bias, ctx.out_dtype = eps, bias is not None, out_dtype
         return y
@@ -74,6 +78,10 @@
     def backward(ctx, dy):
         x, weight, stats = ctx.saved_tensors
         B, L, C = x.shape
+        native = _lib.native_nodes()
+        if native is not None:
+            dx, dwb = native.layer_norm_cm_bwd(x, weight, stats, dy, ctx.eps, ITYPE[ctx.out_dtype], ctx.has_bias)
+            return dx, dwb[:C], (dwb[C:] if ctx.has_bias else None), None, None
         dx = _lib.empty((B, C, L), x.dtype, x.device).transpose(1, 2)
         P = _params(x, ctx.out_dtype, ctx.eps)
         P.dx, P.dx_batch_stride, P.dx_c_stride = dx.data_ptr(), C * L, L
```
